# tudocomp/tudocomp

Measured on AMD Instinct MI355X. Metric: input MB/s end-to-end lcpcomp+huffman, higher is better.
Workload: dtype u32; 1 GPU; lcpcomp(coder=huff,threshold=2,flatten=1,comp=arrays) on 2000000000 B english text (SURVEY 8d generator, seed 42): pinned host text -> H2D -> kernels + host Huffman table -> D2H -> stream in pinned host memory, all timed; bytes_per_gpu=2000000000, parallelism=single GPU

## Files before the change

### include/tdc_gpu.h

```cpp
#ifndef TDC_GPU_H
#define TDC_GPU_H

#include <stddef.h>
#include <stdint.h>

#ifdef __cplusplus
extern "C" {
#endif

typedef enum {
    TDC_GPU_OK = 0,
    TDC_GPU_ERR_HIP = -1,
    TDC_GPU_ERR_ARG = -2,
    TDC_GPU_ERR_NO_SENTINEL = -3,
    TDC_GPU_ERR_TOO_LARGE = -4,
    TDC_GPU_ERR_OOM = -5,
    TDC_GPU_ERR_UNSUPPORTED = -6,
    TDC_GPU_ERR_INTERNAL = -7
} tdc_gpu_status;

enum { TDC_GPU_CODER_HUFF = 0, TDC_GPU_CODER_GAMMA = 1, TDC_GPU_CODER_ARITH = 2, TDC_GPU_CODER_ASCII = 3, TDC_GPU_CODER_SLE = 4,
       TDC_GPU_CODER_BIT = 5 , TDC_GPU_CODER_DELTA = 6  };
#define TDC_GPU_CODER_SLE_K(K) (TDC_GPU_CODER_SLE | ((K) << 8))
enum { TDC_GPU_COMP_ARRAYS = 0, TDC_GPU_COMP_PLCPPEAKS = 1, TDC_GPU_COMP_MAXLCP = 2, TDC_GPU_COMP_HEAP = 3 };

typedef struct tdc_gpu_ctx tdc_gpu_ctx;

typedef struct {
    uint64_t n;
    uint64_t out_len;
    uint64_t factors;
    uint64_t maxlcp;
    uint64_t entries;
    uint64_t num_flattened;
    uint64_t max_depth_lb;
    uint64_t flen_min, flen_max, fdist_max;
    uint64_t pushes;
    uint32_t sa_rounds;
    uint32_t sa_init_syms;
    uint32_t levels;
    uint32_t mis_rounds;
    uint32_t flatten_rounds;
    uint32_t sigma;
    uint64_t sa_sorted_elems;
    uint64_t arena_bytes;
    float ms_h2d, ms_sa, ms_phi, ms_plcp, ms_factorize, ms_flatten, ms_encode, ms_d2h, ms_total;
    uint32_t small_levels;
    uint32_t purges;
    uint32_t window_pass;
    uint32_t window_lcut;
    uint32_t sa_key_words;
    uint32_t sa_text_rounds;
    uint32_t sa_mode;
    uint32_t sa_overlapped;
    uint32_t eager_levels;
    uint32_t eager_phases;
    uint32_t sa_star_chains;
    uint32_t probes;
    uint32_t max_push_targets;
    uint64_t d2h_early;
    uint32_t pipe_stages;
    uint32_t pipe_dev;
    uint64_t pipe_len[8];
    float    pipe_ms[8];
    uint32_t ranges_early;
    uint32_t len_rounds;
    uint64_t rules;
    uint64_t replaced;
    uint32_t tie_rounds;
    uint32_t rebuilds;
    float ms_round_first, ms_round_last, ms_round_tie;
    float reserved1;
} tdc_gpu_stats;

int  tdc_gpu_ctx_create(int device, tdc_gpu_ctx** ctx);
void tdc_gpu_ctx_destroy(tdc_gpu_ctx* ctx);
int tdc_gpu_ctx_set_option(tdc_gpu_ctx* ctx, const char* name, long value);
int tdc_gpu_option_count(void);
const char* tdc_gpu_option_name(int i);
int  tdc_gpu_ctx_reserve(tdc_gpu_ctx* ctx, size_t n);
size_t tdc_gpu_arena_bytes(size_t n);
int  tdc_gpu_device_memory(int device, size_t* free_bytes, size_t* total_bytes);
int  tdc_gpu_ctx_set_profiling(tdc_gpu_ctx* ctx, int enabled);
void tdc_gpu_ctx_reset_profile(tdc_gpu_ctx* ctx);
const char* tdc_gpu_ctx_kernel_profile(const tdc_gpu_ctx* ctx, int idx, double* ms, uint64_t* launches, uint64_t* bytes);
const char* tdc_gpu_strerror(int status);
const char* tdc_gpu_last_error(const tdc_gpu_ctx* ctx);
void tdc_gpu_free(void* p);

int tdc_gpu_lcpcomp_compress(tdc_gpu_ctx* ctx, const uint8_t* text, size_t n, uint32_t threshold, int flatten,
                             int coder, uint8_t** out, size_t* out_len, tdc_gpu_stats* stats);
int tdc_gpu_lcpcomp_compress_comp(tdc_gpu_ctx* ctx, const uint8_t* text, size_t n, uint32_t threshold, int flatten, int coder,
                                  int comp, uint8_t** out, size_t* out_len, tdc_gpu_stats* stats);

int tdc_gpu_lcpcomp_compress_into(tdc_gpu_ctx* ctx, const uint8_t* text, size_t n, uint32_t threshold, int flatten, int coder,
                                  int comp, uint8_t* out, size_t out_cap, size_t* out_len, tdc_gpu_stats* stats);
int tdc_gpu_lcpcomp_compress_keep(tdc_gpu_ctx* ctx, const uint8_t* text, size_t n, uint32_t threshold, int flatten, int coder,
                                  int comp, size_t* out_len, tdc_gpu_stats* stats);
int tdc_gpu_stream_fetch(tdc_gpu_ctx* ctx, uint8_t* dst, size_t cap, size_t* len);
int tdc_gpu_stream_fetch_dev(tdc_gpu_ctx* ctx, void* d_dst, size_t cap, size_t* len);
int tdc_gpu_host_register(void* p, size_t bytes);
int tdc_gpu_host_unregister(void* p);
void* tdc_gpu_host_alloc(size_t bytes);
void  tdc_gpu_host_free(void* p);

int tdc_gpu_lcpcomp_compress_raw(tdc_gpu_ctx* ctx, const uint8_t* data, size_t n, uint32_t threshold, int flatten,
                                 int coder, uint8_t** out, size_t* out_len, tdc_gpu_stats* stats);
int tdc_gpu_lcpcomp_compress_dev(tdc_gpu_ctx* ctx, const void* d_text, size_t n, uint32_t threshold, int flatten,
                                 int coder, void* d_out, size_t out_cap, size_t* out_len, tdc_gpu_stats* stats);
size_t tdc_gpu_lcpcomp_bound(size_t n);
size_t tdc_gpu_lcpcomp_bound_coder(size_t n, int coder);

size_t tdc_gpu_blocks_count(size_t n, size_t block_size);
int tdc_gpu_blocks_compress(const int* devices, int ndev, const uint8_t* data, size_t n, size_t block_size, uint32_t threshold,
                            int flatten, int coder, uint8_t** out, size_t* out_len, tdc_gpu_stats* per_block);
int tdc_gpu_blocks_decompress(tdc_gpu_ctx* ctx, const uint8_t* container, size_t len, int coder, uint8_t** out, size_t* out_len);
int tdc_gpu_device_count(void);

int tdc_gpu_lz78_compress(tdc_gpu_ctx* ctx, const uint8_t* in, size_t n, int coder, uint8_t** out, size_t* out_len,
                          tdc_gpu_stats* stats);

int tdc_gpu_lzss_lcp_compress(tdc_gpu_ctx* ctx, const uint8_t* text, size_t n, uint32_t threshold, int coder,
                              uint8_t** out, size_t* out_len, tdc_gpu_stats* stats);
int tdc_gpu_lzss_lcp_compress_into(tdc_gpu_ctx* ctx, const uint8_t* text, size_t n, uint32_t threshold, int coder,
                                   uint8_t* out, size_t out_cap, size_t* out_len, tdc_gpu_stats* stats);
size_t tdc_gpu_lzss_lcp_bound(size_t n, int coder);
int tdc_gpu_lzss_lcp_decompress(tdc_gpu_ctx* ctx, const uint8_t* stream, size_t len, int coder, uint8_t** out, size_t* out_len,
                                uint64_t* factors, uint32_t* rounds);
int tdc_gpu_lzss_lcp_decompress_into(tdc_gpu_ctx* ctx, const uint8_t* stream, size_t len, int coder, uint8_t* out, size_t out_cap,
                                     size_t* out_len, uint64_t* factors, uint32_t* rounds);
int tdc_gpu_lzss_lcp_factorize(tdc_gpu_ctx* ctx, const uint8_t* text, size_t n, uint32_t threshold,
                               uint32_t** pos, uint32_t** src, uint32_t** len, size_t* z);

int tdc_gpu_sort_pairs_u64(tdc_gpu_ctx* ctx, uint64_t* keys, uint32_t* vals, size_t n, int algo);
int tdc_gpu_suffix_array(tdc_gpu_ctx* ctx, const uint8_t* text, size_t n, uint32_t* sa, uint32_t* isa);
int tdc_gpu_textds(tdc_gpu_ctx* ctx, const uint8_t* text, size_t n, uint32_t* sa, uint32_t* isa, uint32_t* phi,
                   uint32_t* plcp, uint32_t* lcp, uint32_t* maxlcp);
int tdc_gpu_lcpcomp_factorize(tdc_gpu_ctx* ctx, const uint8_t* text, size_t n, uint32_t threshold, int flatten,
                              uint32_t** pos, uint32_t** src, uint32_t** len, size_t* z, tdc_gpu_stats* stats);
int tdc_gpu_flatten(tdc_gpu_ctx* ctx, size_t n, const uint32_t* pos, uint32_t* src, const uint32_t* len, size_t z,
                    uint64_t* num_flattened, uint64_t* max_depth_lb);
int tdc_gpu_prim_scan(tdc_gpu_ctx* ctx, int op, void* data, size_t n, int in_place, void* total);
int tdc_gpu_prim_sort_pairs(tdc_gpu_ctx* ctx, int kind, void* keys, uint32_t* vals, size_t n, int begin_bit, int end_bit);
int tdc_gpu_prim_bucketed_scatter(tdc_gpu_ctx* ctx, const uint32_t* idx, const uint32_t* val, size_t m, uint32_t* dst, size_t n_dst,
                                  uint32_t fill, int permutation, int second_tmp, int offset);
int tdc_gpu_prim_msd_partition(tdc_gpu_ctx* ctx, uint32_t* idx, uint32_t* val, size_t m, int bits, int db);
int tdc_gpu_prim_select(tdc_gpu_ctx* ctx, const uint8_t* cls, uint8_t want, size_t m, const uint32_t* srcA, const uint64_t* srcB,
                        uint32_t fillA, uint64_t fillB, uint32_t* outA, uint64_t* outB, uint32_t* count);
int tdc_gpu_prim_select_counts(tdc_gpu_ctx* ctx, const uint8_t* cls, uint8_t want, size_t m, const uint32_t* srcA, const uint32_t* tile_counts,
                               uint32_t fillA, uint32_t* outA, uint32_t* count);
int tdc_gpu_prim_mark_orbit(tdc_gpu_ctx* ctx, const uint32_t* next, size_t n, uint8_t* mark);
int tdc_gpu_prim_tile_entries(tdc_gpu_ctx* ctx, const uint16_t* exit0, size_t ntiles, uint32_t states, uint16_t* entry0);
int tdc_gpu_prim_arena_fill(tdc_gpu_ctx* ctx, int byte, uint64_t* base, uint64_t* size);

int tdc_gpu_lcpcomp_decompress(tdc_gpu_ctx* ctx, const uint8_t* stream, size_t len, uint8_t** out, size_t* out_len,
// ... 133 lines not shown
```

### tudocomp_amd/_native.py

```python
import ctypes
import os

_HERE = os.path.dirname(os.path.abspath(__file__))
LIB_PATH = os.environ.get("TDC_GPU_LIB") or os.path.join(_HERE, "lib", "libtdc_gpu.so")

SYMBOLS = [
    "tdc_gpu_ctx_create", "tdc_gpu_ctx_destroy", "tdc_gpu_ctx_reserve", "tdc_gpu_strerror", "tdc_gpu_last_error",
    "tdc_gpu_ctx_set_profiling", "tdc_gpu_ctx_reset_profile", "tdc_gpu_ctx_kernel_profile",
    "tdc_gpu_free", "tdc_gpu_lcpcomp_compress", "tdc_gpu_lcpcomp_compress_raw", "tdc_gpu_lcpcomp_compress_dev",
    "tdc_gpu_lcpcomp_bound", "tdc_gpu_lcpcomp_bound_coder", "tdc_gpu_lcpcomp_compress_into", "tdc_gpu_host_alloc", "tdc_gpu_host_free",
    "tdc_gpu_lz78_compress", "tdc_gpu_lzss_lcp_compress", "tdc_gpu_lzss_lcp_factorize",
    "tdc_gpu_sort_pairs_u64", "tdc_gpu_suffix_array", "tdc_gpu_textds", "tdc_gpu_lcpcomp_factorize", "tdc_gpu_flatten", "tdc_gpu_encode_huff",
    "tdc_gpu_prim_scan", "tdc_gpu_prim_sort_pairs", "tdc_gpu_prim_bucketed_scatter", "tdc_gpu_prim_msd_partition", "tdc_gpu_prim_select", "tdc_gpu_prim_select_counts",
    "tdc_gpu_prim_mark_orbit", "tdc_gpu_prim_tile_entries", "tdc_gpu_prim_arena_fill",
    "tdc_gpu_lcpcomp_decompress",
    "tdc_gpu_lcpcomp_compress_comp",
    "tdc_gpu_encode_arith",
    "tdc_gpu_encode_ascii",
    "tdc_gpu_encode_sle",
    "tdc_gpu_lcpcomp_decompress_coder", "tdc_gpu_ctx_last_decode_on_device", "tdc_gpu_lcpcomp_decompress_into",
    "tdc_gpu_ctx_set_option", "tdc_gpu_option_count", "tdc_gpu_option_name", "tdc_escape", "tdc_unescape", "tdc_lz78_factors", "tdc_huffman_table", "tdc_huffman_selfcheck", "tdc_gpu_blocks_count", "tdc_gpu_blocks_compress", "tdc_gpu_blocks_decompress", "tdc_gpu_device_count", "tdc_gen_english", "tdc_gen_dna",
    "tdc_gpu_arena_bytes", "tdc_gpu_device_memory",
    "tdc_gpu_lcpcomp_compress_keep", "tdc_gpu_stream_fetch", "tdc_gpu_stream_fetch_dev", "tdc_gpu_host_register", "tdc_gpu_host_unregister",
    "tdc_gpu_lz78_decompress", "tdc_gpu_lz78_decompress_into",
    "tdc_gpu_bwt_compress", "tdc_gpu_bwt_compress_into", "tdc_gpu_bwt_decompress", "tdc_gpu_bwt_decompress_into", "tdc_gpu_bwt_inverse_stage",
    "tdc_gpu_pipeline_bound", "tdc_gpu_pipeline_compress", "tdc_gpu_pipeline_compress_into", "tdc_gpu_pipeline_decompress",
    "tdc_gpu_pipeline_decompress_into", "tdc_gpu_pipeline_decompress_stats", "tdc_rle_decode", "tdc_mtf_decode", "tdc_huff_decode_literals", "tdc_sle_decode",
    "tdc_gpu_lzw_compress", "tdc_gpu_lzw_decompress", "tdc_gpu_lzw_decompress_into", "tdc_lzw_factors", "tdc_lzw_decode",
    "tdc_gpu_lzss_lcp_compress_into", "tdc_gpu_lzss_lcp_bound", "tdc_gpu_lzss_lcp_decompress", "tdc_gpu_lzss_lcp_decompress_into", "tdc_lzss_decode",
    "tdc_gpu_lzss_sw_compress", "tdc_gpu_lzss_sw_compress_into", "tdc_gpu_lzss_sw_bound", "tdc_gpu_lzss_sw_factorize", "tdc_lzss_sw_factors",
    "tdc_lzss_sw_decode", "tdc_gpu_lzss_sw_decompress", "tdc_gpu_lzss_sw_decompress_into",
    "tdc_gpu_lzss_sw_compress_batch", "tdc_gpu_lzss_sw_batch_bound", "tdc_gpu_lzss_sw_decompress_batch",
    "tdc_gpu_lzw_compress_batch", "tdc_gpu_lzw_batch_bound", "tdc_gpu_lz78_compress_batch", "tdc_gpu_lz78_batch_bound", "tdc_gpu_lz_parse_batch",
    "tdc_gpu_lzw_decompress_batch", "tdc_gpu_lz78_decompress_batch",
    "tdc_gpu_repair_compress", "tdc_gpu_repair_compress_into", "tdc_gpu_repair_bound", "tdc_gpu_repair_grammar", "tdc_gpu_repair_decompress",
    "tdc_gpu_repair_decompress_into", "tdc_gpu_repair_decompress_stats", "tdc_repair_grammar", "tdc_repair_decode",
]


class Stats(ctypes.Structure):
    _fields_ = (
        [(k, ctypes.c_uint64) for k in ("n", "out_len", "factors", "maxlcp", "entries", "num_flattened", "max_depth_lb",
                                        "flen_min", "flen_max", "fdist_max", "pushes")] +
        [(k, ctypes.c_uint32) for k in ("sa_rounds", "sa_init_syms", "levels", "mis_rounds", "flatten_rounds", "sigma")] +
        [(k, ctypes.c_uint64) for k in ("sa_sorted_elems", "arena_bytes")] +
        [(k, ctypes.c_float) for k in ("ms_h2d", "ms_sa", "ms_phi", "ms_plcp", "ms_factorize", "ms_flatten", "ms_encode",
                                       "ms_d2h", "ms_total")] +
        [(k, ctypes.c_uint32) for k in ("small_levels", "purges", "window_pass", "window_lcut",
                                        "sa_key_words", "sa_text_rounds", "sa_mode", "sa_overlapped", "eager_levels", "eager_phases", "sa_star_chains",
                                        "probes", "max_push_targets")] +
        [("d2h_early", ctypes.c_uint64)] +
        [("pipe_stages", ctypes.c_uint32), ("pipe_dev", ctypes.c_uint32), ("pipe_len", ctypes.c_uint64 * 8), ("pipe_ms", ctypes.c_float * 8),
         ("ranges_early", ctypes.c_uint32), ("len_rounds", ctypes.c_uint32),
         ("rules", ctypes.c_uint64), ("replaced", ctypes.c_uint64), ("tie_rounds", ctypes.c_uint32), ("rebuilds", ctypes.c_uint32),
         ("ms_round_first", ctypes.c_float), ("ms_round_last", ctypes.c_float), ("ms_round_tie", ctypes.c_float), ("reserved1", ctypes.c_float)])

    def as_dict(self):
        d = {k: getattr(self, k) for k, _ in self._fields_}
        d["pipe_len"] = list(self.pipe_len)[:self.pipe_stages]
        d["pipe_ms"] = list(self.pipe_ms)[:self.pipe_stages]
        return d


class Stage(ctypes.Structure):
    _fields_ = [("kind", ctypes.c_int), ("param", ctypes.c_uint64)]


_lib = None


def load():
    global _lib
    if _lib is not None:
        return _lib
    if not os.path.exists(LIB_PATH):
        raise RuntimeError("tudocomp_amd: %s is missing -- build it with `make -C tudocomp_amd/csrc` "
                           "(there is no CPU fallback)" % LIB_PATH)
    L = ctypes.CDLL(LIB_PATH)
    vp, sz, u32, i32 = ctypes.c_void_p, ctypes.c_size_t, ctypes.c_uint32, ctypes.c_int
    pvp, psz = ctypes.POINTER(vp), ctypes.POINTER(sz)
    L.tdc_gpu_ctx_create.argtypes = [i32, pvp]
    L.tdc_gpu_ctx_destroy.argtypes = [vp]
    L.tdc_gpu_ctx_destroy.restype = None
    L.tdc_gpu_ctx_reserve.argtypes = [vp, sz]
    L.tdc_gpu_ctx_set_profiling.argtypes = [vp, i32]
    L.tdc_gpu_ctx_reset_profile.argtypes = [vp]
    L.tdc_gpu_ctx_reset_profile.restype = None
    L.tdc_gpu_ctx_kernel_profile.argtypes = [vp, i32, ctypes.POINTER(ctypes.c_double), ctypes.POINTER(ctypes.c_uint64),
                                             ctypes.POINTER(ctypes.c_uint64)]
    L.tdc_gpu_ctx_kernel_profile.restype = ctypes.c_char_p
    L.tdc_gpu_strerror.argtypes = [i32]
    L.tdc_gpu_strerror.restype = ctypes.c_char_p
    L.tdc_gpu_last_error.argtypes = [vp]
    L.tdc_gpu_last_error.restype = ctypes.c_char_p
    L.tdc_gpu_free.argtypes = [vp]
    L.tdc_gpu_free.restype = None
    L.tdc_gpu_lcpcomp_compress.argtypes = [vp, vp, sz, u32, i32, i32, pvp, psz, ctypes.POINTER(Stats)]
    L.tdc_gpu_lcpcomp_compress_comp.argtypes = [vp, vp, sz, u32, i32, i32, i32, pvp, psz, ctypes.POINTER(Stats)]
    L.tdc_gpu_lcpcomp_compress_raw.argtypes = [vp, vp, sz, u32, i32, i32, pvp, psz, ctypes.POINTER(Stats)]
    L.tdc_gpu_lcpcomp_compress_dev.argtypes = [vp, vp, sz, u32, i32, i32, vp, sz, psz, ctypes.POINTER(Stats)]
    L.tdc_gpu_lz78_compress.argtypes = [vp, vp, sz, i32, pvp, psz, ctypes.POINTER(Stats)]
    L.tdc_gpu_lzss_lcp_compress.argtypes = [vp, vp, sz, u32, i32, pvp, psz, ctypes.POINTER(Stats)]
    L.tdc_gpu_lzss_lcp_compress_into.argtypes = [vp, vp, sz, u32, i32, vp, sz, psz, ctypes.POINTER(Stats)]
    L.tdc_gpu_lzss_lcp_bound.argtypes = [sz, i32]
    L.tdc_gpu_lzss_lcp_bound.restype = sz
    L.tdc_gpu_lzss_lcp_decompress.argtypes = [vp, vp, sz, i32, pvp, psz, ctypes.POINTER(ctypes.c_uint64), ctypes.POINTER(ctypes.c_uint32)]
    L.tdc_gpu_lzss_lcp_decompress_into.argtypes = [vp, vp, sz, i32, vp, sz, psz, ctypes.POINTER(ctypes.c_uint64), ctypes.POINTER(ctypes.c_uint32)]
    L.tdc_lzss_decode.argtypes = [vp, sz, i32, vp, sz, psz]
    L.tdc_gpu_lzss_lcp_factorize.argtypes = [vp, vp, sz, u32, pvp, pvp, pvp, psz]
    L.tdc_gpu_arena_bytes.argtypes = [sz]
    L.tdc_gpu_arena_bytes.restype = sz
    L.tdc_gpu_device_memory.argtypes = [i32, psz, psz]
    L.tdc_gpu_lcpcomp_bound.argtypes = [sz]
    L.tdc_gpu_lcpcomp_bound.restype = sz
    L.tdc_gpu_lcpcomp_bound_coder.argtypes = [sz, i32]
    L.tdc_gpu_lcpcomp_bound_coder.restype = sz
    L.tdc_gpu_lcpcomp_compress_into.argtypes = [vp, vp, sz, u32, i32, i32, i32, vp, sz, psz, ctypes.POINTER(Stats)]
    L.tdc_gpu_lcpcomp_compress_keep.argtypes = [vp, vp, sz, u32, i32, i32, i32, psz, ctypes.POINTER(Stats)]
    L.tdc_gpu_stream_fetch.argtypes = [vp, vp, sz, psz]
    L.tdc_gpu_stream_fetch_dev.argtypes = [vp, vp, sz, psz]
    L.tdc_gpu_ctx_last_decode_on_device.argtypes = [vp]
    L.tdc_gpu_lcpcomp_decompress_into.argtypes = [vp, vp, sz, i32, vp, sz, psz, ctypes.POINTER(ctypes.c_uint64), ctypes.POINTER(ctypes.c_uint32)]
    L.tdc_gpu_host_register.argtypes = [vp, sz]
    L.tdc_gpu_host_unregister.argtypes = [vp]
    L.tdc_gpu_blocks_count.argtypes = [sz, sz]
    L.tdc_gpu_blocks_count.restype = sz
    L.tdc_gpu_blocks_compress.argtypes = [ctypes.POINTER(i32), i32, vp, sz, sz, u32, i32, i32, pvp, psz, ctypes.POINTER(Stats)]
    L.tdc_gpu_blocks_decompress.argtypes = [vp, vp, sz, i32, pvp, psz]
    L.tdc_gpu_host_alloc.argtypes = [sz]
    L.tdc_gpu_host_alloc.restype = vp
    L.tdc_gpu_host_free.argtypes = [vp]
    L.tdc_gpu_host_free.restype = None
    L.tdc_gpu_sort_pairs_u64.argtypes = [vp, vp, vp, sz, i32]
    L.tdc_gpu_prim_scan.argtypes = [vp, i32, vp, sz, i32, vp]
    L.tdc_gpu_prim_sort_pairs.argtypes = [vp, i32, vp, vp, sz, i32, i32]
    L.tdc_gpu_prim_bucketed_scatter.argtypes = [vp, vp, vp, sz, vp, sz, u32, i32, i32, i32]
    L.tdc_gpu_prim_msd_partition.argtypes = [vp, vp, vp, sz, i32, i32]
    L.tdc_gpu_prim_select.argtypes = [vp, vp, ctypes.c_uint8, sz, vp, vp, u32, ctypes.c_uint64, vp, vp, ctypes.POINTER(u32)]
# ... 83 lines not shown
```

### tudocomp_amd/csrc/api_compress.hip

```cpp
#include "api.hpp"
#include "bitsink.hpp"

#include <vector>

using namespace tdc;

namespace tdc {

void validate_device_text(Ctx& c, const u8* d_text, size_t n) {
    if (!(c.hist_ptr == d_text && c.hist_n == n)) {
        const size_t mark = c.arena.mark();
        u32* d_hist = c.arena.get<u32>(256);
        HIP_TRY(hipMemsetAsync(d_hist, 0, 256 * sizeof(u32), c.stream));
        text_histogram_add(c, d_text, n, d_hist);
        text_histogram_finish(c, d_text, n, d_hist);
        c.arena.release(mark);
    }
    u8 last = 1;
    HIP_TRY(hipMemcpyAsync(&last, d_text + n - 1, 1, hipMemcpyDeviceToHost, c.stream));
    HIP_TRY(hipStreamSynchronize(c.stream));
    const u32 zeros = c.hist_cache[0];
    if (last != 0) throw ArgError{TDC_GPU_ERR_NO_SENTINEL, "text does not end with a 0 sentinel"};
    if (zeros != 1) throw ArgError{TDC_GPU_ERR_ARG, "text contains 0 bytes besides the sentinel (escape the input first)"};
}

static bool early_is_planned(const Ctx& c, size_t n, u32 threshold, int flatten, int strategy, int enc_coder, const u8* d_text) {
    return strategy == TDC_GPU_COMP_ARRAYS && flatten && enc_coder == 0 && d_text && c.enc_early && c.enc_rec && c.huff_ok &&
           n >= (c.enc_early >= 2 ? (size_t)1 : ((size_t)1 << 20)) && threshold >= 2;
}

void run_textds(Ctx& c, const u8* d_text, size_t n, DevArrays& A, tdc_gpu_stats* st, Events* ev, bool want_phi, const CandWant* cw) {
    A.sa = c.arena.get<u32>(n);
    A.isa = c.arena.get<u32>(n);
    A.phi = nullptr;
    A.plcp = c.arena.get<u32>(n);
    u32* d_max = c.arena.get<u32>(1);
    SAStats ss;
    SAExtra ex;
    ex.lcp8 = c.arena.get<u8>(n + 64);
    const int e0 = ev ? ev->tick() : 0;
    build_suffix_array(c, d_text, n, A.sa, A.isa, &ss, &ex);
    const int e1 = ev ? ev->tick() : 0;
    int e2;
    if (!(ex.mode == 1 && !want_phi && c.phi_lazy)) A.phi = c.arena.get<u32>(n);
    if (ex.mode == 1) {
        CandFused* cf = nullptr;
        if (cw && c.fused_cand && !A.phi && fused_scatter_has_image(c, n)) {
            cf = &A.cand;
            cf->threshold = cw->threshold;
            cf->lcut = factorize_arrays_lcut0(c, n, cw->threshold);
            cf->cls = c.arena.get<u8>(n);
            if (cf->lcut) cf->res8 = c.arena.get<u8>(n);
            if (cw->flen8) cf->flen8 = A.fs.flen8 = c.arena.get<u8>(n + 64); else cf->flen = A.fs.flen = c.arena.get<u32>(n);
            if (c.sel_tile_counts) cf->tilecnt = c.arena.get<u32>(cdiv(n, SEL_TILE_CLASSES));
            cf->acc = c.arena.get<u32>((size_t)CF_COPIES * CF_ACC);
            cf->lvlhist = c.arena.get<u32>(128);
            cf->entries = cf->lvlhist + 64;
        }
        build_isa_phi_plcp_fused(c, A.sa, ex.lcp8, n, A.isa, A.phi, A.plcp, d_max, cf);
        e2 = ev ? ev->tick() : 0;
    } else {
        build_phi(c, A.sa, n, A.phi);
        e2 = ev ? ev->tick() : 0;
        build_plcp(c, d_text, n, A.phi, A.plcp, d_max);
    }
    const int e3 = ev ? ev->tick() : 0;
    A.maxlcp = c.read(d_max);
    if (st) {
        st->maxlcp = A.maxlcp;
        sa_stats(st, ss, &ex);
        if (ev) { ev->span(&st->ms_sa, e0, e1); ev->span(&st->ms_phi, e1, e2); ev->span(&st->ms_plcp, e2, e3); }
    }
}

constexpr size_t FLAT_CHUNK_MIN = (size_t)16 << 20;
constexpr size_t FLAT_CHUNK_MAX = 8;

void run_factorize(Ctx& c, size_t n, DevArrays& A, u32 threshold, int flatten, tdc_gpu_stats* st, Events* ev, int strategy,
                   int enc_coder, const u8* d_text) {
    if (!A.fs.flen) A.fs.flen = c.arena.get<u32>(n);
    A.fs.owner = c.arena.get<u32>(n);
    A.fs.fsrc = c.arena.get<u32>(n);
    A.fs.fpos = c.arena.get<u32>(n);
    A.fs.flenl = threshold >= 2 ? A.fs.fpos + (n + 1) / 2 : nullptr;
    A.fs.cls = c.arena.get<u8>(n + 64);
    const bool early_planned = early_is_planned(c, n, threshold, flatten, strategy, enc_coder, d_text);
    if (early_planned && c.flen_bytes && !A.fs.flen8) A.fs.flen8 = c.arena.get<u8>(n + 64);
    A.fs.want_owner_rem = early_planned ? (u32)c.owner_rem : 0u;
    FactorizeStats fz;
    FlattenStats fl;
    const int e0 = ev ? ev->tick() : 0;
    if (strategy == TDC_GPU_COMP_PLCPPEAKS) plcp_peaks_factorize(c, n, A.phi, A.plcp, threshold, A.fs, &fz.factors);
    else if (strategy == TDC_GPU_COMP_MAXLCP) factorize_max_lcp(c, n, A.isa, A.phi, A.plcp, A.maxlcp, threshold, A.fs, &fz);
    else if (strategy == TDC_GPU_COMP_HEAP) factorize_max_heap(c, n, A.sa, A.isa, A.plcp, A.maxlcp, threshold, A.fs, &fz);
    else factorize_arrays(c, n, A.sa, A.isa, A.phi, A.plcp, A.maxlcp, threshold, A.fs, &fz, A.cand.filled ? &A.cand : nullptr);
    const int e1 = ev ? ev->tick() : 0;
    const bool early = flatten && enc_coder == 0 && d_text && c.enc_early && c.huff_ok && n >= (c.enc_early >= 2 ? (size_t)1 : ((size_t)1 << 20)) &&
                       A.fs.have_list && A.fs.have_cls && A.fs.flenl && A.fs.nfact > 0;
    if (!early) expand_flen8(c, n, A.fs);
    if (early) {
        A.early = encode_early_reserve(c, n, c.enc_rec ? A.fs.nfact : 0);
        u32 K = c.flatten_chunks ? (u32)c.flatten_chunks : (u32)std::min<size_t>(A.fs.nfact / FLAT_CHUNK_MIN, FLAT_CHUNK_MAX);
        K = flatten_chunk_count(K, A.fs.nfact);
        const bool packed = K >= 2 && encode_early_chunks(c, n, A.fs, A.early, K, align_up(encode_bound_coder(n, enc_coder) + 16, 8));
        if (!packed && c.flatten_chunks < 2) K = 1;
        c.wait_for(c.copy_stream, c.stream);
        flatten_factors(c, n, A.fs, &fl, [&](int round) {
            StreamSwap sw(c, c.copy_stream);
            if (round == 1 || round == 2) encode_early_run(c, d_text, n, A.fs, enc_coder, A.early, false);
            else if (round == 0) encode_early_run(c, d_text, n, A.fs, enc_coder, A.early, true);
        }, c.enc_rec ? encode_early_rec(A.early) : nullptr, K,
        packed ? std::function<void(u32, size_t)>([&](u32 k, size_t) { encode_early_chunk_done(c, d_text, n, A.fs, A.early, k); }) : std::function<void(u32, size_t)>());
    } else if (flatten) {
        flatten_factors(c, n, A.fs, &fl);
    } else {
        materialize_sources(c, n, A.fs);
    }
    const int e2 = ev ? ev->tick() : 0;
    if (st) {
        st->factors = fz.factors; st->entries = fz.entries; st->pushes = fz.pushes;
        st->levels = fz.levels; st->mis_rounds = fz.rounds; st->small_levels = fz.small_levels; st->purges = fz.purges; st->window_pass = fz.window_pass; st->window_lcut = fz.window_lcut; st->eager_levels = fz.eager_levels; st->eager_phases = fz.eager_phases;
        st->probes = fz.probes; st->max_push_targets = fz.max_push_targets;
        st->num_flattened = fl.num_flattened; st->max_depth_lb = fl.max_depth_lb; st->flatten_rounds = fl.rounds;
        st->ranges_early = A.early ? encode_early_packed(A.early) : 0u;
        if (ev) { ev->span(&st->ms_factorize, e0, e1); ev->span(&st->ms_flatten, e1, e2); }
    }
}

u8* TextUpload::send(const uint8_t* text, size_t n) {
    if (n < ((size_t)1 << 26)) return upload_plain(c, text, n);
    u8* d_text = c.arena.get<u8>(n + 64);
    u32* d_hist = c.arena.get<u32>(256);
    HIP_TRY(hipMemsetAsync(d_hist, 0, 256 * sizeof(u32), c.stream));
    c.wait_for(c.copy_stream, c.stream);
    const bool try_pre = c.wsort_overlap && c.wpre && wsort_applicable(c, n);
    const size_t CH = try_pre ? (size_t)c.upload_chunks : 8;
    std::vector<size_t> coff;
    {
        std::vector<double> w(CH, 1.0);
        if (try_pre) {
            const size_t T = std::min<size_t>((size_t)c.upload_tail_n, CH - 1);
            double f = 1.0;
            for (size_t k = 0; k < T; ++k) { f *= (double)c.upload_tail_pct / 100.0; w[CH - T + k] = f; }
        }
        double tot = 0; for (double x : w) tot += x;
        coff.push_back(0);
        double acc = 0;
        for (size_t k = 0; k + 1 < CH; ++k) {
            acc += w[k];
            size_t o = ((size_t)((double)n * (acc / tot)) + 4095) & ~(size_t)4095;
            if (o <= coff.back()) o = coff.back() + 4096;
            if (o >= n) break;
            coff.push_back(o);
        }
        coff.push_back(n);
    }
    const size_t nch = coff.size() - 1;
    if (nch > Ctx::CHUNK_EVENTS) throw HipError{hipErrorUnknown, "upload: more chunks than chunk events", (int)__LINE__};
    size_t queued = 0;
    auto queue_copies = [&](size_t upto) {
        for (; queued < nch && queued < upto; ++queued) {
            const size_t off = coff[queued] + (queued ? 64 : 0), end = std::min(coff[queued + 1] + 64, n);
            if (end > off) HIP_TRY(hipMemcpyAsync(d_text + off, text + off, end - off, hipMemcpyHostToDevice, c.copy_stream));
            HIP_TRY(hipEventRecord(c.ev_chunk[queued], c.copy_stream));
            (void)hipStreamQuery(c.copy_stream);
        }
    };
    bool pre_on = false;
    for (size_t q = 0; q < nch; ++q) {
        const size_t off = coff[q], len = coff[q + 1] - off;
        queue_copies(q + 4);
        HIP_TRY(hipStreamWaitEvent(c.stream, c.ev_chunk[q], 0));
        text_histogram_add(c, d_text + off, len, d_hist);
        if (q == 0 && try_pre) {
            u32 h0[256];
            c.read_n(d_hist, h0, 256);
            pre_on = wsort_pre_begin(c, *c.wpre, d_text, n, coff.data(), (u32)nch, h0);
            if (!pre_on) c.arena.release_top();
        }
        if (pre_on) wsort_pre_chunk(c, *c.wpre, (u32)q);
    }
    text_histogram_finish(c, d_text, n, d_hist);
    if (pre_on) {
        wsort_pre_finish(c, *c.wpre, c.hist_cache);
        if (!c.wpre->active) c.arena.release_top();
    }
    return d_text;
}

struct HostBuf {
    void* p = nullptr;
    explicit HostBuf(size_t bytes) : p(malloc(bytes ? bytes : 1)) { if (!p) throw std::bad_alloc(); }
    ~HostBuf() { free(p); }
    template <typename T> T* release() { T* r = (T*)p; p = nullptr; return r; }
    HostBuf(const HostBuf&) = delete;
    HostBuf& operator=(const HostBuf&) = delete;
};

void download_factors(Ctx& c, size_t n, const FactorSpace& fs, Events& ev, uint32_t** pos, uint32_t** src, uint32_t** len, size_t* z) {
    u32* d_pos = c.arena.get<u32>(n), *d_src = c.arena.get<u32>(n), *d_len = c.arena.get<u32>(n);
    const size_t cnt = extract_factors(c, n, fs, d_pos, d_src, d_len, n);
    HostBuf hp(cnt * 4), hs(cnt * 4), hl(cnt * 4);
    if (cnt) {
        HIP_TRY(hipMemcpyAsync(hp.p, d_pos, cnt * 4, hipMemcpyDeviceToHost, c.stream));
        HIP_TRY(hipMemcpyAsync(hs.p, d_src, cnt * 4, hipMemcpyDeviceToHost, c.stream));
        HIP_TRY(hipMemcpyAsync(hl.p, d_len, cnt * 4, hipMemcpyDeviceToHost, c.stream));
    }
// ... 623 lines not shown
```

### tudocomp_amd/csrc/api_ctx.hip

```cpp
#include "api.hpp"
#include "huffman_host.hpp"

#include <strings.h>
#include <ctype.h>

using namespace tdc;

namespace tdc {

int lcpcomp_enc_coder(int coder) {
    const int base = coder & 0xFF, k = coder >> 8;
    if (base == TDC_GPU_CODER_SLE) {
        if (k < 0 || k > 7) throw ArgError{TDC_GPU_ERR_ARG, "sle: kmer must be in 1..7"};
        return 3 | ((k ? k : 3) << 8);
    }
    if (k == 0 && base == TDC_GPU_CODER_HUFF) return 0;
    if (k == 0 && base == TDC_GPU_CODER_ARITH) return 1;
    if (k == 0 && base == TDC_GPU_CODER_ASCII) return 2;
    throw ArgError{TDC_GPU_ERR_UNSUPPORTED, "lcpcomp: coder must be huff, arithmetic, ascii or sle"};
}

void reserve_arena(Ctx& c, size_t bytes) {
    if (c.arena.size < bytes) {
        size_t fr = 0, tot = 0;
// ... 25 lines not shown
        default: return "unknown status";
    }
}

const char* tdc_gpu_last_error(const tdc_gpu_ctx* ctx) { return ctx ? ctx->last_error.c_str() : ""; }

void tdc_gpu_free(void* p) { free(p); }

namespace {
struct OptionDef { const char* name; void (*set)(Ctx&, long); };
inline int clampi(long v, long lo, long hi) { return (int)(v < lo ? lo : (v > hi ? hi : v)); }
const OptionDef OPTIONS[] = {
    { "fastread",         [](Ctx& c, long v) { c.fast_read = v ? 1 : 0; } },
    { "sa_local",         [](Ctx& c, long v) { c.sa_local_sort = (int)v; } },
    { "radix_waves",      [](Ctx& c, long v) { c.radix_waves = v == 8 ? 8 : 4; } },
    { "window_lcut",      [](Ctx& c, long v) { c.window_lcut = clampi(v, 0, 63); } },
    { "window_halo",      [](Ctx& c, long v) { c.window_halo = clampi(v, 0, 2048); } },
    { "dec_seg",          [](Ctx& c, long v) { c.dec_seg = v < 4096 ? 4096 : (v > (1l << 30) ? (size_t)1 << 30 : (size_t)v); } },
    { "dec_lean",         [](Ctx& c, long v) { c.dec_lean = v != 0; } },
    { "dec_parse",        [](Ctx& c, long v) { c.dec_parse = clampi(v, 0, 2); } },
    { "dec_done",         [](Ctx& c, long v) { c.dec_done = v != 0; } },
    { "dec_log",          [](Ctx& c, long v) { c.dec_log = v != 0; } },
    { "bwt_log",          [](Ctx& c, long v) { c.bwt_log = v != 0; } },
    { "pipe_log",         [](Ctx& c, long v) { c.pipe_log = v != 0; } },
    { "window_force_fail",[](Ctx& c, long v) { c.window_force_fail = v ? 1 : 0; } },
    { "window_large",     [](Ctx& c, long v) { c.window_large_lists = v ? 1 : 0; } },
    { "window_src",       [](Ctx& c, long v) { c.window_src = v ? 1 : 0; } },
    { "plcp_samples",     [](Ctx& c, long v) { c.plcp_samples = v != 0; } },
    { "small_pipeline",   [](Ctx& c, long v) { c.small_pipeline = v != 0; } },
    { "small_big",        [](Ctx& c, long v) { c.small_big = (int)v; } },
    { "small_prof",       [](Ctx& c, long v) { c.small_prof = v != 0; } },
    { "phi_lazy",         [](Ctx& c, long v) { c.phi_lazy = v != 0; } },
    { "fs_pair",          [](Ctx& c, long v) { c.fs_pair = v != 0; } },
    { "enc_early",        [](Ctx& c, long v) { c.enc_early = (int)v; } },
    { "owner_rem",        [](Ctx& c, long v) { c.owner_rem = (int)std::min<long>(std::max<long>(v, 0), 8); } },
    { "enc_rec",          [](Ctx& c, long v) { c.enc_rec = v != 0; } },
    { "level_purge",      [](Ctx& c, long v) { c.level_purge = v != 0; } },
    { "level_log",        [](Ctx& c, long v) { c.level_log = v != 0; } },
    { "eager",            [](Ctx& c, long v) { c.eager_levels = v != 0; } },
    { "eager_dump",       [](Ctx& c, long v) { c.eager_dump = v != 0; } },
    { "flen_bytes",       [](Ctx& c, long v) { c.flen_bytes = v != 0; } },
    { "flatten_steps",    [](Ctx& c, long v) { c.flatten_steps = v <= 0 ? (1 << 30) : clampi(v, 1, 1 << 30); } },
    { "flatten_growth",   [](Ctx& c, long v) { c.flatten_growth = clampi(v, 2, 1 << 20); } },
    { "sa_refine",        [](Ctx& c, long v) { c.sa_refine = v != 0; } },
    { "sa_pairs",         [](Ctx& c, long v) { c.sa_pairs = v != 0; } },
    { "sa_stars",         [](Ctx& c, long v) { c.sa_stars = v != 0; } },
    { "sa_fused_init",    [](Ctx& c, long v) { c.sa_fused_init = v != 0; } },
    { "sa_init_syms",     [](Ctx& c, long v) { c.sa_init_syms = clampi(v, 0, 64); } },
    { "radix_lds",        [](Ctx& c, long v) { c.radix_lds = (v >= 0 && v <= 2) ? (int)v : 2; } },
    { "xcd_remap",        [](Ctx& c, long v) { c.xcd_remap = (v >= 0 && v <= 2) ? (int)v : 0; } },
    { "bucket_scatter",   [](Ctx& c, long v) { c.bucket_scatter = v ? 1 : 0; } },
    { "ssort",            [](Ctx& c, long v) { c.ssort = v ? 1 : 0; } },
    { "ssort_levels",     [](Ctx& c, long v) { c.ssort_levels = (v >= 1 && v <= 3) ? (int)v : 0; } },
    { "msd_partition",    [](Ctx& c, long v) { c.msd_partition = v ? 1 : 0; } },
    { "wsort",            [](Ctx& c, long v) { c.wsort = v ? 1 : 0; } },
    { "wsort_min",        [](Ctx& c, long v) { c.wsort_min = v < 4096 ? 4096 : (size_t)v; } },
    { "wsort_syms",       [](Ctx& c, long v) { c.wsort_syms = (v >= 4 && v <= 64) ? (int)v : 0; } },
    { "wsort_kw",         [](Ctx& c, long v) { c.wsort_kw = (v == 1 || v == 2) ? (int)v : 0; } },
    { "wsort_rounds",     [](Ctx& c, long v) { c.wsort_rounds = clampi(v, 0, 100); } },
    { "wsort_smallrun",   [](Ctx& c, long v) { c.wsort_small = v ? 1 : 0; } },
    { "wsort_overlap",    [](Ctx& c, long v) { c.wsort_overlap = v ? 1 : 0; } },
    { "wsort_predig",     [](Ctx& c, long v) { c.wsort_predig = v ? 1 : 0; } },
    { "wsort_prehist",    [](Ctx& c, long v) { c.wsort_prehist = v ? 1 : 0; } },
    { "sa_seg_bigcap",    [](Ctx& c, long v) { c.sa_seg_bigcap = clampi(v, 0, 65536); } },
    { "sa_seg_rounds",    [](Ctx& c, long v) { c.sa_seg_rounds = clampi(v, 0, 2); } },
    { "wsort_run_streams",[](Ctx& c, long v) { c.wsort_run_streams = v != 0; } },
    { "wsort_predig_skip",[](Ctx& c, long v) { c.wsort_predig_skip = clampi(v, 0, 24); } },
    { "wsort_fuse",       [](Ctx& c, long v) { c.wsort_fuse = v ? 1 : 0; } },
    { "wsort_order",      [](Ctx& c, long v) { c.wsort_order = v ? 1 : 0; } },
    { "wsort_two",        [](Ctx& c, long v) { c.wsort_two = (v >= 0 && v <= 2) ? (int)v : 0; } },
    { "wsort_leaf",       [](Ctx& c, long v) { c.wsort_leaf = v == 1024 ? 1024 : 2048; } },
    { "wsort_pack",       [](Ctx& c, long v) { c.wsort_pack = (v == 1024 || v == 4096) ? (int)v : 2048; } },
    { "wsort_cmax",       [](Ctx& c, long v) { c.wsort_cmax = clampi(v, 8, 64); } },
    { "wsort_log",        [](Ctx& c, long v) { c.wsort_log = v != 0; } },
    { "upload_chunks",    [](Ctx& c, long v) { c.upload_chunks = clampi(v, 4, 24); } },
    { "upload_tail_n",    [](Ctx& c, long v) { c.upload_tail_n = clampi(v, 0, 12); } },
    { "upload_tail_pct",  [](Ctx& c, long v) { c.upload_tail_pct = clampi(v, 30, 100); } },
    { "arena_log",        [](Ctx& c, long v) { c.arena_log = v != 0; } },
};
constexpr size_t NOPTIONS = sizeof(OPTIONS) / sizeof(OPTIONS[0]);
const OptionDef FOLD_OPTIONS[] = {
    { "fused_cand",       [](Ctx& c, long v) { c.fused_cand = v != 0; } },
    { "sel_tile_counts",  [](Ctx& c, long v) { c.sel_tile_counts = v != 0; } },
    { "flatten_chunks",   [](Ctx& c, long v) { c.flatten_chunks = clampi(v, 0, (long)FLATTEN_MAX_CHUNKS); } },
    { "repair_recount",   [](Ctx& c, long v) { c.repair_recount = v != 0; } },
    { "repair_table_bits",[](Ctx& c, long v) { c.repair_table_bits = v == 0 ? 0 : clampi(v, 8, 30); } },
    { "repair_log",       [](Ctx& c, long v) { c.repair_log = v != 0; } },
    { "repair_dec_rounds",[](Ctx& c, long v) { c.repair_dec_rounds = clampi(v, 1, 1 << 24); } },
    { "lz_batch_hash_bits",[](Ctx& c, long v) { c.lz_batch_hash_bits = clampi(v, 0, 24); } },
};
constexpr size_t NFOLD = sizeof(FOLD_OPTIONS) / sizeof(FOLD_OPTIONS[0]);
const OptionDef* find_option(const char* name) {
    if (!name) return nullptr;
    if (!strncasecmp(name, "TDC_GPU_", 8)) name += 8;
    for (size_t i = 0; i < NOPTIONS; ++i) if (!strcasecmp(name, OPTIONS[i].name)) return &OPTIONS[i];
    for (size_t i = 0; i < NFOLD; ++i) if (!strcasecmp(name, FOLD_OPTIONS[i].name)) return &FOLD_OPTIONS[i];
    return nullptr;
}
void apply_env_options(tdc_gpu_ctx* ctx) {
    const char* on = getenv("TDC_GPU_DEBUG_KNOBS");
    if (!on || atoi(on) == 0) return;
    for (size_t i = 0; i < NOPTIONS + NFOLD; ++i) {
        const OptionDef& o = i < NOPTIONS ? OPTIONS[i] : FOLD_OPTIONS[i - NOPTIONS];
        char var[64] = "TDC_GPU_";
        size_t k = 8;
        for (const char* q = o.name; *q && k + 1 < sizeof(var); ++q) var[k++] = (char)toupper((unsigned char)*q);
        var[k] = 0;
        if (const char* m = getenv(var)) o.set(ctx->c, atol(m));
    }
}
}

int tdc_gpu_ctx_set_option(tdc_gpu_ctx* ctx, const char* name, long value) {
    if (!ctx) return TDC_GPU_ERR_ARG;
    const OptionDef* o = find_option(name);
    if (!o) return TDC_GPU_ERR_ARG;
    o->set(ctx->c, value);
    return TDC_GPU_OK;
}
int tdc_gpu_option_count(void) { return (int)NOPTIONS; }
const char* tdc_gpu_option_name(int i) { return (i >= 0 && (size_t)i < NOPTIONS) ? OPTIONS[i].name : nullptr; }

int tdc_gpu_ctx_create(int device, tdc_gpu_ctx** out) {
    if (!out) return TDC_GPU_ERR_ARG;
    *out = nullptr;
    int count = 0;
    if (hipGetDeviceCount(&count) != hipSuccess || count <= 0) { (void)hipGetLastError(); return TDC_GPU_ERR_HIP; }
    if (device < 0 || device >= count) return TDC_GPU_ERR_ARG;
    tdc_gpu_ctx* ctx = new (std::nothrow) tdc_gpu_ctx();
    if (!ctx) return TDC_GPU_ERR_OOM;
    ctx->c.huff_ok = huffman_selfcheck();
    ctx->c.device = device;
    ctx->c.wpre = &ctx->pre;
    DeviceGuard dg(device);
    try {
        HIP_TRY(dg.enter());
        HIP_TRY(hipStreamCreateWithFlags(&ctx->c.stream, hipStreamNonBlocking));
        for (auto& e : ctx->c.ev) HIP_TRY(hipEventCreate(&e));
        HIP_TRY(hipStreamCreateWithFlags(&ctx->c.copy_stream, hipStreamNonBlocking));
        {
            int lo = 0, hi = 0;
            if (hipDeviceGetStreamPriorityRange(&lo, &hi) != hipSuccess) { lo = 0; (void)hipGetLastError(); }
            if (hipStreamCreateWithPriority(&ctx->c.aux_stream, hipStreamNonBlocking, lo) != hipSuccess) { ctx->c.aux_stream = nullptr; (void)hipGetLastError(); }
        }
        HIP_TRY(hipEventCreateWithFlags(&ctx->c.ev_join, hipEventDisableTiming));
        HIP_TRY(hipEventCreateWithFlags(&ctx->c.ev_dig2, hipEventDisableTiming));
        for (auto& e : ctx->c.ev_chunk) HIP_TRY(hipEventCreateWithFlags(&e, hipEventDisableTiming));
        ctx->c.pinned_size = 4096;
        HIP_TRY(hipHostMalloc(&ctx->c.pinned, ctx->c.pinned_size, hipHostMallocDefault));
        HIP_TRY(hipHostMalloc((void**)&ctx->c.pinned_hdr, Ctx::PINNED_HDR, hipHostMallocDefault));
        if (ctx->c.fast_read) {
            void* zc = nullptr;
            if (hipHostMalloc(&zc, (size_t)Ctx::ZC_WORDS * Ctx::ZC_BLOCKS * 4, hipHostMallocMapped | hipHostMallocCoherent) == hipSuccess) {
                void* dv = nullptr;
                if (hipHostGetDevicePointer(&dv, zc, 0) == hipSuccess) { ctx->c.zc_host = (u32*)zc; ctx->c.zc_dev = (u32*)dv; memset(zc, 0, (size_t)Ctx::ZC_WORDS * Ctx::ZC_BLOCKS * 4); }
                else { (void)hipHostFree(zc); (void)hipGetLastError(); }
            } else (void)hipGetLastError();
        }
        HIP_TRY(hipMalloc((void**)&ctx->c.d_err, 256));
        HIP_TRY(hipMemset(ctx->c.d_err, 0, 256));
        apply_env_options(ctx);
    } catch (const HipError&) {
        (void)hipGetLastError();
        tdc_gpu_ctx_destroy(ctx);
        return TDC_GPU_ERR_HIP;
    }
    *out = ctx;
// ... 141 lines not shown
```

### tudocomp_amd/csrc/common.hpp

```cpp
#pragma once

#include <hip/hip_runtime.h>
#include <stdint.h>
#include <stddef.h>
#include <stdio.h>
#include <string.h>

namespace tdc {

typedef uint8_t  u8;
typedef uint32_t u32;
typedef uint16_t u16;
typedef uint64_t u64;

constexpr u32 NONE32 = 0xFFFFFFFFu;
constexpr int WAVE = 64;

enum {
    TDC_OK = 0,
    TDC_ERR_HIP = -1,
    TDC_ERR_ARG = -2,
    TDC_ERR_NO_SENTINEL = -3,
    TDC_ERR_TOO_LARGE = -4,
    TDC_ERR_OOM = -5,
// ... 34 lines not shown
        if (top > high) high = top;
        return base + off;
    }
    template <typename T> T* get(size_t count) { return (T*)alloc(count * sizeof(T)); }
    void* alloc_top(size_t bytes) {
        if (bytes + top_hi + 256 > size) throw HipError{hipErrorOutOfMemory, "arena (top)", (int)__LINE__};
        const size_t off = (size - top_hi - bytes) & ~(size_t)255;
        if (off < top) throw HipError{hipErrorOutOfMemory, "arena (top)", (int)__LINE__};
        top_hi = size - off;
        return base + off;
    }
    template <typename T> T* get_top(size_t count) { return (T*)alloc_top(count * sizeof(T)); }
    void release_top() { top_hi = 0; }
    size_t mark() const { return top; }
    void release(size_t m) { top = m; }
};

enum KernelClass {
    K_RS_SCATTER_U64 = 0, K_RS_SCATTER_U32, K_RS_COUNT, K_SCAN,
    K_SA_RANK_SCATTER, K_SA_BUILD_KEYS, K_PHI, K_PLCP, K_CAND,
    K_LEVEL_INIT, K_MIS_ROUND, K_RESOLVE, K_PUSH, K_APPLY, K_POOL, K_SMALL_LEVEL, K_WINDOW_LEVELS,
    K_FLATTEN_ROUND, K_ENC_GAPS, K_ENC_HIST, K_ENC_TILE_BITS, K_ENC_PACK, K_EXTRACT, K_SS_LEAF, K_SA_LOCAL_SORT, K_WINDOW_SCATTER,
    K_WS_LEAF_SORT, K_WS_LEAF_COUNT, K_WS_RUN, K_FS_IMAGE,
    K_CLASS_COUNT
};

struct KernelProfile {
    double ms = 0;
    u64 launches = 0;
    u64 bytes = 0;
};

#ifdef __HIPCC__
static __global__ void publish_words_kernel(const uint32_t* __restrict__ src, uint32_t nwords, uint32_t* host_dst, uint32_t* host_flag,
                                            uint32_t seq) {
    for (uint32_t i = threadIdx.x; i < nwords; i += blockDim.x)
        __hip_atomic_store(&host_dst[i], src[i], __ATOMIC_RELAXED, __HIP_MEMORY_SCOPE_SYSTEM);
    __syncthreads();
    if (threadIdx.x == 0) {
        __threadfence_system();
        __hip_atomic_store(host_flag, seq, __ATOMIC_RELEASE, __HIP_MEMORY_SCOPE_SYSTEM);
    }
}
#endif

struct Ctx {
    int device = 0;
    hipStream_t stream = nullptr;
    Arena arena;
    hipEvent_t ev[16] = {};
    void* pinned = nullptr;
    size_t pinned_size = 0;
    void* pinned_tab = nullptr;
    size_t pinned_tab_size = 0;
    u8* pinned_hdr = nullptr;
    static constexpr size_t PINNED_HDR = 65536;
    void* pinned_table(size_t bytes) {
        if (pinned_tab_size < bytes) {
            if (pinned_tab) { (void)hipHostFree(pinned_tab); pinned_tab = nullptr; pinned_tab_size = 0; }
            HIP_TRY(hipHostMalloc(&pinned_tab, bytes, hipHostMallocDefault));
            pinned_tab_size = bytes;
        }
        return pinned_tab;
    }
    static constexpr u32 ZC_SEG_OFF = 1040, ZC_WORDS = 1040 + 16384;
    static constexpr u32 ZC_BLOCKS = 3;
    u32* zc_host = nullptr;
    u32* zc_dev = nullptr;
    u32 zc_seq = 0;
    int fast_read = 1;
    u32* d_err = nullptr;
    int sa_local_sort = 1;
    int radix_waves = 4;
    int plcp_samples = 1;
    bool huff_ok = true;
    int flen_bytes = 1;
    int eager_levels = 1;
    int level_purge = 1;
    int enc_rec = 1;
    int owner_rem = 8;
    int enc_early = 1;
    int fused_cand = 1;
    int sel_tile_counts = 1;
    int fs_pair = 1;
    int small_big = 1;
    int small_pipeline = 1;
    int sa_pairs = 1;
    int sa_stars = 1;
    int sa_refine = 1;
    int sa_fused_init = 1;
    int radix_lds = 1;
    int xcd_remap = 1;
    int window_src = 1;
    int window_lcut = 56;
    int window_halo = 320;
    size_t dec_seg = 0;
    bool phi_lazy = true;
    int dec_lean = 1;
    int dec_parse = 1;
    int window_force_fail = 0;
    int window_large_lists = 0;
    int ssort = 1;
    int ssort_levels = 0;
    int wsort = 1;
    size_t wsort_min = (size_t)1 << 20;
    int wsort_syms = 0;
    int wsort_kw = 0;
    int wsort_rounds = 24;
    int wsort_cmax = 24;
    int wsort_overlap = 1;
    int wsort_prehist = 1;
    bool wsort_count_nonheads = true;
    int sa_seg_bigcap = 65536;
    int sa_seg_rounds = 2;
    int wsort_run_streams = 1;
    int wsort_predig_skip = 4;
    int wsort_predig = 1;
    int wsort_two = 0;
    int wsort_leaf = 2048;
    int wsort_pack = 1024;
    int wsort_order = 1;
    int wsort_fuse = 1;
    int wsort_small = 0;
    int msd_partition = 1;
    int bucket_scatter = 1;
    int upload_tail_n = 3, upload_tail_pct = 60;
    int upload_chunks = 16;
    int flatten_steps = 1;
    int flatten_growth = 8;
    int flatten_chunks = 0;
    int sa_init_syms = 0;
    int dec_done = 1;
    int repair_recount = 0;
    int repair_table_bits = 0;
    int repair_log = 0;
    int repair_dec_rounds = 1024;
    int lz_batch_hash_bits = 0;
    int dec_log = 0, bwt_log = 0, pipe_log = 0, level_log = 0, wsort_log = 0, eager_dump = 0, small_prof = 0, arena_log = 0;

    u32 hist_cache[256] = {};
    const u8* hist_ptr = nullptr;
    size_t hist_n = 0;
    hipStream_t copy_stream = nullptr;
    hipStream_t aux_stream = nullptr;
    hipEvent_t ev_join = nullptr;
    static constexpr size_t CHUNK_EVENTS = 32;
    hipEvent_t ev_chunk[CHUNK_EVENTS] = {};
    hipEvent_t ev_dig2 = nullptr;
    struct WPre* wpre = nullptr;
    u8* d2h_host = nullptr;
    size_t d2h_cap = 0;
    size_t d2h_done = 0;

    bool profiling = false;
    KernelProfile kprof[K_CLASS_COUNT];
    struct Pending { hipEvent_t a, b; int cls; u64 bytes; };
    Pending* pend = nullptr;
    int npend = 0, pend_cap = 0;
    hipEvent_t* ev_pool = nullptr;
    int ev_pool_size = 0, ev_pool_used = 0;

    int prof_begin(int cls, u64 bytes) {
        if (!profiling || npend >= pend_cap || ev_pool_used + 2 > ev_pool_size) return -1;
        Pending& p = pend[npend];
        p.a = ev_pool[ev_pool_used++]; p.b = ev_pool[ev_pool_used++]; p.cls = cls; p.bytes = bytes;
        HIP_TRY(hipEventRecord(p.a, stream));
// ... 291 lines not shown
```

### tudocomp_amd/csrc/encode.hip

```cpp
#include "stages.hpp"
#include "bytestages.hpp"
#include "bitsink.hpp"
#include "prim.hpp"
#include "huffman_host.hpp"
#include "arith.hpp"
#include "decode.hpp"

#include <string.h>
#include <algorithm>
#include <vector>

namespace tdc {

struct CodeTable {
    u64 code[256];
    u8 len[256];
};

struct EncParams {
    u32 W, lbits, dbits, flen_min;
    u32 raw_literals;
    u32 ascii;
    u32 uni;
};
// ... 498 lines not shown
        build_huffman_table(h_hist, &ht);
        write_huffman_header(hw, ht);
    } else {
        ArithModel am;
        if (!arith_build_model(h_hist, &am, hw))
            throw HipError{hipErrorInvalidValue, "arithmetic coder: all literal bytes >= 1 are absent (the reference divides by zero)", -1};
        ArithPlan plan;
        arith_prepare(c, text, n, plain_owner(fs), am, &plan);
        E.A.litidx = plan.litidx; E.A.amark = plan.amark; E.A.fval = plan.fval; E.A.lc_index = plan.lc_index; E.A.pp_lb = plan.pp_lb;
    }
    EncParams& P = E.P;
    P.W = bits_for(n);
    P.lbits = bits_for((u64)h_sc.flen_max - (u64)h_sc.flen_min);
    P.dbits = bits_for(h_sc.fdist_max);
    P.flen_min = h_sc.flen_min;
    P.raw_literals = (ht.sigma <= 1) ? 1u : 0u;
    P.ascii = (coder == 2) ? 1u : 0u;
    P.uni = coder == 5 ? (u32)ENC_GAMMA : coder == 6 ? (u32)ENC_DELTA : 0u;
    if (P.uni) {
        const u64 fields[4] = { (u64)n, h_sc.flen_min, h_sc.flen_max, h_sc.fdist_max };
        auto gamma = [&](u64 v) { const unsigned b = bits_for(v); hw.write_int(0, b); hw.write_bit(true); hw.write_int(v, b); };
        for (u64 v : fields) {
            if (P.uni == (u32)ENC_GAMMA) gamma(v);
            else { gamma(bits_for(v)); hw.write_int(v, bits_for(v)); }
        }
    } else if (coder == 2) {
        const u64 fields[4] = { (u64)n, h_sc.flen_min, h_sc.flen_max, h_sc.fdist_max };
        for (u64 v : fields) {
            char tmp[24]; int k = 0;
            do { tmp[k++] = (char)('0' + v % 10); v /= 10; } while (v);
            while (k) hw.write_int((u8)tmp[--k], 8);
            hw.write_int(':', 8);
        }
    } else {
        hw.write_int(n, 32);
        hw.write_int(h_sc.flen_min, P.W);
        hw.write_int(h_sc.flen_max, P.W);
        hw.write_int(h_sc.fdist_max, P.W);
    }
    E.base_bits = hw.nbits;
    memcpy(E.tab.code, ht.code_of, sizeof(E.tab.code));
    memcpy(E.tab.len, ht.len_of, sizeof(E.tab.len));

    const unsigned tiles = E.tiles;
    u64* tile_bits = E.tile_bits;
    {
        Ctx::ProfScope prof(c, K_ENC_TILE_BITS, (u64)n * 9);
        if (P.uni == (u32)ENC_GAMMA) tile_bits_kernel<ENC_GAMMA><<<tiles, 256, 0, s>>>(text, plain_owner(fs), fs.flen, fs.fsrc, n, E.tab, P, E.A, tile_bits);
        else if (P.uni == (u32)ENC_DELTA) tile_bits_kernel<ENC_DELTA><<<tiles, 256, 0, s>>>(text, plain_owner(fs), fs.flen, fs.fsrc, n, E.tab, P, E.A, tile_bits);
        else if (P.ascii) tile_bits_kernel<ENC_ASCII><<<tiles, 256, 0, s>>>(text, plain_owner(fs), fs.flen, fs.fsrc, n, E.tab, P, E.A, tile_bits);
        else if (fs.have_cls) tile_bits_cls_kernel<<<tiles, 256, 0, s>>>(text, fs.cls, n, E.tab, P, E.A, tile_bits, E.tile_rank);
        else         tile_bits_kernel<ENC_TAB><<<tiles, 256, 0, s>>>(text, plain_owner(fs), fs.flen, fs.fsrc, n, E.tab, P, E.A, tile_bits);
        LAUNCH_CHECK();
    }
    exclusive_sum_u64(c, tile_bits, tile_bits, tiles, E.d_tp);
    if (E.tile_rank) exclusive_sum_u32(c, E.tile_rank, E.tile_rank, tiles, nullptr);
    E.may_overlap = may_overlap(c, E);
    pick_u64_kernel<<<1, 64, 0, s>>>(tile_bits, E.end, E.nb, E.d_tp + 1);
    LAUNCH_CHECK();
    E.seq_b = c.publish_async(E.d_tp, (1 + PACK_CH) * sizeof(u64), 2);
    E.step = 2;
}

static void encode_step_c(Ctx& c, EncodeEarly& E) {
    u64 h_tp[1 + PACK_CH] = { 0 };
    if (E.seq_b) c.publish_wait(E.seq_b, h_tp, sizeof(h_tp), 2); else c.read_n(E.d_tp, h_tp, 1 + PACK_CH);
    const bool may_overlap = E.may_overlap;
    E.total_bits = E.base_bits + h_tp[0];
    E.out_len = bit_stream_len(E.total_bits);
    E.overlap = may_overlap && E.out_len <= c.d2h_cap;
    for (u32 q = 0; q < PACK_CH; ++q) E.h_end[q] = h_tp[1 + q];
    E.step = 3;
    E.done = true;
}

static void encode_first_half(Ctx& c, const u8* text, size_t n, FactorSpace& fs, int coder, EncodeEarly& E, bool finish = true) {
    do {
        if (E.step == 0) encode_step_a(c, text, n, fs, E);
        else if (E.step == 1) encode_step_b(c, text, n, fs, coder, E);
        else if (E.step == 2) encode_step_c(c, E);
    } while (finish && E.step < 3);
}

EncodeEarly* encode_early_reserve(Ctx& c, size_t n, size_t z_rec) {
    EncodeEarly* E = new EncodeEarly();
    try { encode_reserve(c, n, *E, z_rec); } catch (...) { delete E; throw; }
    return E;
}
void* encode_early_rec(EncodeEarly* E) { return E->rec; }
void encode_early_run(Ctx& c, const u8* text, size_t n, FactorSpace fs, int coder, EncodeEarly* E, bool finish) { encode_first_half(c, text, n, fs, coder, *E, finish); }
void encode_early_free(EncodeEarly* E) { delete E; }

static void pack_begin(Ctx& c, hipStream_t ps, EncodeEarly& E, u8* d_out) {
    if (E.begun) return;
    const HostBitWriter& hw = E.hw;
    HIP_TRY(hipMemsetAsync(d_out, 0, bit_stream_padded(E.out_len), ps));
    if (c.pinned_hdr && hw.bytes.size() <= Ctx::PINNED_HDR) {
        memcpy(c.pinned_hdr, hw.bytes.data(), hw.bytes.size());
        HIP_TRY(hipMemcpyAsync(d_out, c.pinned_hdr, hw.bytes.size(), hipMemcpyHostToDevice, ps));
    } else HIP_TRY(hipMemcpyAsync(d_out, hw.bytes.data(), hw.bytes.size(), hipMemcpyHostToDevice, ps));
    E.begun = true;
}
static void pack_upto(Ctx& c, hipStream_t ps, hipStream_t cs, const u8* text, size_t n, const FactorSpace& fs, EncodeEarly& E, u8* d_out, u32 upto) {
    if (upto <= E.q_done) return;
    const EncParams& P = E.P;
    const ArithDev& A = E.A;
    const CodeTable& tab = E.tab;
    const u64 base_bits = E.base_bits;
    const u64* tile_bits = E.tile_bits;
    const u32 t0 = E.q_done ? E.end.end[E.q_done - 1] : 0u, t1 = upto == E.nb ? E.tiles : E.end.end[upto - 1];
    if (t1 > t0) {
        if (P.uni == (u32)ENC_GAMMA) pack_kernel<ENC_GAMMA><<<t1 - t0, 256, 0, ps>>>(text, plain_owner(fs), fs.flen, fs.fsrc, n, tab, P, A, tile_bits, base_bits, (u64*)d_out, t0);
        else if (P.uni == (u32)ENC_DELTA) pack_kernel<ENC_DELTA><<<t1 - t0, 256, 0, ps>>>(text, plain_owner(fs), fs.flen, fs.fsrc, n, tab, P, A, tile_bits, base_bits, (u64*)d_out, t0);
        else if (P.ascii) pack_kernel<ENC_ASCII><<<t1 - t0, 256, 0, ps>>>(text, plain_owner(fs), fs.flen, fs.fsrc, n, tab, P, A, tile_bits, base_bits, (u64*)d_out, t0);
        else if (fs.have_cls && E.rec) pack_cls_kernel<true><<<t1 - t0, 256, 0, ps>>>(text, fs.cls, fs.flen, fs.fsrc, n, tab, P, A, tile_bits, base_bits, (u64*)d_out, t0, E.rec, E.tile_rank, (u32)E.z_rec);
        else if (fs.have_cls) pack_cls_kernel<false><<<t1 - t0, 256, 0, ps>>>(text, fs.cls, fs.flen, fs.fsrc, n, tab, P, A, tile_bits, base_bits, (u64*)d_out, t0, nullptr, nullptr, 0u);
        else         pack_kernel<ENC_TAB><<<t1 - t0, 256, 0, ps>>>(text, plain_owner(fs), fs.flen, fs.fsrc, n, tab, P, A, tile_bits, base_bits, (u64*)d_out, t0);
        LAUNCH_CHECK();
    }
    E.q_done = upto;
    if (E.overlap && upto < E.nb) {
        const size_t safe = (size_t)((base_bits + E.h_end[upto - 1]) / 64) * 8;
        bool room = true;
        if (E.by_rank && E.ncopy >= PACK_AHEAD) room = hipEventQuery(c.ev_chunk[PACK_CH + E.ncopy - PACK_AHEAD]) == hipSuccess;
        if (safe > E.copied && room) {
            c.wait_for(cs, ps);
            HIP_TRY(hipMemcpyAsync(c.d2h_host + E.copied, d_out + E.copied, safe - E.copied, hipMemcpyDeviceToHost, cs));
            if (E.by_rank) {
                HIP_TRY(hipEventRecord(c.ev_chunk[PACK_CH + E.ncopy++], cs));
                (void)hipStreamQuery(cs);
            }
            E.copied = safe;
        }
    }
}

bool encode_early_chunks(Ctx& c, size_t n, const FactorSpace& fs, EncodeEarly* e, u32 K, size_t out_cap) {
    EncodeEarly& E = *e;
    const size_t z = fs.nfact;
    if (K < 2 || K > FLATTEN_MAX_CHUNKS || K > z || !fs.have_list || !E.rec || E.z_rec != z || E.step != 0 || !c.aux_stream || !c.pinned_hdr || !may_overlap(c, E)) return false;
    E.d_out = c.arena.get<u8>(out_cap);
    E.out_cap = out_cap;
    u32 h[FLATTEN_MAX_CHUNKS] = { 0 };
    const size_t mark = c.arena.mark();
    u32* d_b = c.arena.get<u32>(FLATTEN_MAX_CHUNKS);
    range_tiles_kernel<<<1, 64, 0, c.stream>>>(fs.fpos, (u32)z, K, d_b);
    LAUNCH_CHECK();
    c.read_n(d_b, h, K - 1);
    c.arena.release(mark);
    for (u32 k = 0; k + 1 < K; ++k) E.end.end[k] = std::min<u32>(h[k], E.tiles);
    for (u32 k = K - 1; k < PACK_CH; ++k) E.end.end[k] = E.tiles;
    E.nb = K;
    E.by_rank = true;
    return true;
}
u8* encode_early_out(EncodeEarly* e, size_t* out_cap) { if (e->d_out && out_cap) *out_cap = e->out_cap; return e->d_out; }
u32 encode_early_packed(const EncodeEarly* e) { return e->by_rank ? e->q_done : 0u; }

void encode_early_chunk_done(Ctx& c, const u8* text, size_t n, const FactorSpace& fs, EncodeEarly* e, u32 k) {
    EncodeEarly& E = *e;
    if (!E.by_rank || k >= E.nb) return;
    HIP_TRY(hipEventRecord(c.ev_chunk[k], c.stream));
    E.q_ready = k + 1;
    if (E.step == 2 && E.seq_b && c.publish_test(E.seq_b, 2)) encode_step_c(c, E);
    if (!E.done || bit_stream_padded(E.out_len) > E.out_cap) return;
    if (E.q_ready == E.nb) return;
    const hipStream_t ps = c.copy_stream, cs = c.aux_stream;
    pack_begin(c, ps, E, E.d_out);
    HIP_TRY(hipStreamWaitEvent(ps, c.ev_chunk[k], 0));
// ... 616 lines not shown
```

### tudocomp_amd/csrc/factorize.hip

```cpp
#include "stages.hpp"
#include "prim.hpp"
#include "factorize_tiles.hpp"
#include "factorize_eager.hpp"

#include <algorithm>
#include <map>
#include <unordered_map>
#include <chrono>
#include <stdlib.h>
#include <vector>

namespace tdc {

enum : u8 { CL_DEAD = 0, CL_LIVE = 1, CL_STALE = 2 };

struct PushSeg { u32 target, start; };
struct GatherSeg { u32 src_off, dst_off; };
constexpr u32 SEG_INLINE = 508;

struct SmallCtl { u32 pool_top, prio_base; };

struct LevelScalars {
    u32 nlive, nstale;
    u32 undecided;
// ... 869 lines not shown
    const u32 i = blockIdx.x * blockDim.x + threadIdx.x;
    if (i >= npush) return;
    const u32 tgt = (u32)(keys[i] >> 32);
    const u32 p = vals[i];
    prio[p] = prio_base + i;
    pool[i] = p;
    if (res8) res8[p] = res8_pushed(tgt);
    if (i == 0 || (u32)(keys[i - 1] >> 32) != tgt) {
        const u32 j = atomicAdd(&sc->nseg, 1u);
        if (j < SEG_INLINE) sc->segs[j] = PushSeg{tgt, i};
        if (j < seg_cap) segs[j] = PushSeg{tgt, i};
    }
}

template <int G>
__global__ __launch_bounds__(256) void apply_kernel(const u32* __restrict__ live, u32 nl, u32 L, size_t n, u64* bm,
                                                     const u32* phi, u32* __restrict__ cur, u32* __restrict__ flen,
                                                     u32* fsrc, LevelScalars* __restrict__ sc, u8* __restrict__ res8, u8* __restrict__ flen8) {
    const u32 i = (blockIdx.x * blockDim.x + threadIdx.x) / G;
    const u32 sub = (G == 1) ? 0u : (threadIdx.x & (G - 1));
    bool sel = false;
    u32 p = 0;
    if (i < nl) { p = live[i]; sel = (bm_state(bm, p) == 2u); }
    if (sel) {
        if (sub == 0) { put_flen(flen, flen8, p, L); if (phi != fsrc) fsrc[p] = phi[p]; }
        for (u32 j = sub; j < L && (size_t)p + j < n; j += G) cur[p + j] = 0;
        const u32 aff = (L < p) ? L : p;
        for (u32 j = sub; j < aff; j += G) {
            u32* q = &cur[p - 1 - j];
            if (*q > j + 1) { if (atomicMin(q, j + 1) > j + 1 && res8) res8[p - 1 - j] = res8_mark(j + 1); }
        }
    }
    if (G > 1) __builtin_amdgcn_wave_barrier();
    if (sel && sub == 0) atomicAnd((unsigned long long*)&bm[p >> 5], ~(3ull << (2 * (p & 31))));
    __shared__ u32 cnt;
    if (threadIdx.x == 0) cnt = 0;
    __syncthreads();
    const u64 b = __ballot(sel && sub == 0);
    if (lane_id() == 0 && b) atomicAdd(&cnt, (u32)__popcll(b));
    __syncthreads();
    if (threadIdx.x == 0 && cnt) atomicAdd(&sc->selected, cnt);
}

u32 factorize_arrays_lcut0(const Ctx& c, size_t n, u32 threshold) {
    if (c.window_lcut <= 0 || n < window_levels_min_text()) return 0;
    const u32 lcut = std::min<u32>((u32)c.window_lcut, window_levels_max_lcut());
    return lcut < threshold ? 0u : lcut;
}

void factorize_arrays(Ctx& c, size_t n, const u32* sa, u32* isa, const u32* phi, u32* plcp, u32 maxlcp, u32 threshold,
                      FactorSpace& fs, FactorizeStats* st, const CandFused* cf) {
    const u32* phi_eff = phi ? phi : fs.fsrc;
    FactorizeStats local;
    if (!st) st = &local;
    *st = FactorizeStats();
    st->maxlcp = maxlcp;
    if (n == 0) return;
    hipStream_t s = c.stream;
    const size_t mark = c.arena.mark();
    const unsigned gn = cdiv(n, 256);
    u32* cur = plcp;
    u32* prio = isa;

    const bool pre = cf && cf->filled;
    if (pre && (phi || cf->threshold != threshold || cf->lcut != factorize_arrays_lcut0(c, n, threshold) || (fs.flen8 ? cf->flen8 != fs.flen8 : cf->flen != fs.flen)))
        throw HipError{hipErrorUnknown, "factorize: the pre-classified candidates belong to another call", (int)__LINE__};
    u8* cls = pre ? cf->cls : c.arena.get<u8>(n);
    u32 lcut = factorize_arrays_lcut0(c, n, threshold);
    if (lcut > maxlcp) lcut = maxlcp;
    if (lcut < threshold) lcut = 0;
    u8* res8 = lcut ? (pre ? cf->res8 : c.arena.get<u8>(n)) : nullptr;
    u32* ckeys[2] = { c.arena.get<u32>(n), c.arena.get<u32>(n) };
    u32* cvals[2] = { c.arena.get<u32>(n), c.arena.get<u32>(n) };
    u32* d_cnt = c.arena.get<u32>(4);
    u32* d_lvlhist = pre ? cf->lvlhist : c.arena.get<u32>(64);
    if (!pre) {
        HIP_TRY(hipMemsetAsync(d_cnt, 0, 4 * sizeof(u32), s));
        HIP_TRY(hipMemsetAsync(d_lvlhist, 0, 64 * sizeof(u32), s));
        Ctx::ProfScope prof(c, K_CAND, (u64)n * (lcut ? 10 : 9) - (fs.flen8 ? (u64)n * 3 : 0));
        cand_class_kernel<<<(gn < 8192u ? gn : 8192u), 256, 0, s>>>(plcp, n, threshold, lcut, cls, fs.flen, res8, d_cnt + 1, lcut ? d_lvlhist : nullptr,
                                                                    phi ? nullptr : sa, isa, fs.fsrc, fs.flen8);
        LAUNCH_CHECK();
    }
    if ((u64)maxlcp + 1 <= threshold || threshold == 0) { c.arena.release(mark); build_owner(c, n, fs); if (!phi) { fs.src_prio = prio; fs.src_sa = sa; fs.src_n = n; } return; }
    const size_t nlev = (size_t)maxlcp + 2;
    u64* rkey = c.arena.get<u64>(n + 2);
    u32* d_segstart = (u32*)rkey;
    u32* d_segend = d_segstart + nlev;
    std::vector<u32> h_segstart(nlev), h_segend(nlev);
    int x = 0;
    size_t cand_count = 0;
    bool first_lists = true;
    auto build_lists = [&](u32 max_level) {
        const bool from_image = pre && first_lists;
        first_lists = false;
        select_by_class(c, cls, 1, n, nullptr, cvals[0], nullptr, nullptr, d_cnt, from_image && c.sel_tile_counts ? cf->tilecnt : nullptr);
        cand_count = c.read(d_cnt);
        if (from_image && !phi && cand_count) {
            Ctx::ProfScope prof(c, K_CAND, (u64)cand_count * 16);
            cand_source_kernel<<<cdiv(cand_count, 256), 256, 0, s>>>(cvals[0], cand_count, sa, isa, n, fs.fsrc);
            LAUNCH_CHECK();
        }
        if (cand_count) {
            Ctx::ProfScope prof(c, K_CAND, (u64)cand_count * 12);
            gather_kernel<<<cdiv(cand_count, 256), 256, 0, s>>>(cvals[0], cand_count, plcp, ckeys[0]);
            LAUNCH_CHECK();
        }
        x = radix_sort_pairs_u32(c, ckeys, cvals, cand_count, 0, (int)bits_for(max_level));
        HIP_TRY(hipMemsetAsync(d_segstart, 0, nlev * sizeof(u32), s));
        HIP_TRY(hipMemsetAsync(d_segend, 0, nlev * sizeof(u32), s));
        if (cand_count) {
            seg_bounds_kernel<<<cdiv(cand_count, 256), 256, 0, s>>>(ckeys[x], cand_count, d_segstart, d_segend);
            LAUNCH_CHECK();
        }
        c.read_n(d_segstart, h_segstart.data(), nlev);
        c.read_n(d_segend, h_segend.data(), nlev);
    };
    build_lists(maxlcp);
    st->entries = c.read(pre ? cf->entries : d_cnt + 1);
    const u32* cand = cvals[x];

    u32* ent = c.arena.get<u32>(n);
    u32* live = c.arena.get<u32>(n);
    u32* stale = c.arena.get<u32>(n);
    const size_t bm_words = n / 32 + 2;
    u64* bm = c.arena.get<u64>(bm_words);
    HIP_TRY(hipMemsetAsync(bm, 0, bm_words * sizeof(u64), s));
    u8* rc = c.arena.get<u8>(n);
    u32* pool = c.arena.get<u32>(n);
    u32* pushed = c.arena.get<u32>(n);
    u32* rval = c.arena.get<u32>(n);
    u64* skeys[2] = { c.arena.get<u64>(n), c.arena.get<u64>(n) };
    u32* svals[2] = { c.arena.get<u32>(n), c.arena.get<u32>(n) };
    LevelScalars* d_sc = (LevelScalars*)c.arena.alloc(sizeof(LevelScalars));
    LevelScalars* d_sc2[2] = { d_sc, (LevelScalars*)c.arena.alloc(sizeof(LevelScalars)) };
    SmallCtl* d_ctl = (SmallCtl*)c.arena.alloc(sizeof(SmallCtl));
    const u32 seg_cap = 1u << 16;
    PushSeg* d_segs = (PushSeg*)c.arena.alloc(sizeof(PushSeg) * seg_cap);
    PushSeg* d_segs2[2] = { d_segs, (PushSeg*)c.arena.alloc(sizeof(PushSeg) * seg_cap) };
    u32 force_general_level = NONE32;
    std::vector<PushSeg> h_segs(seg_cap);
    LevelScalars h_sc;

    const u32 gtab_cap = 1u << 16;
    GatherSeg* d_gtab = (GatherSeg*)c.arena.alloc(sizeof(GatherSeg) * gtab_cap);
    GatherSeg* h_gtab = (GatherSeg*)c.pinned_table(sizeof(GatherSeg) * gtab_cap);
    GatherSeg* d_hgtab = nullptr;
    if (hipHostGetDevicePointer((void**)&d_hgtab, h_gtab, 0) != hipSuccess) { d_hgtab = nullptr; (void)hipGetLastError(); }
    struct PoolSeg { u32 off, cnt; };
    struct LevelLists {
        std::vector<std::vector<PoolSeg>> flat;
        std::unordered_map<u32, std::vector<PoolSeg>> m;
        void init(size_t levels) { if (levels <= ((size_t)1 << 20)) flat.resize(levels); }
        const std::vector<PoolSeg>& get(u32 lv) const {
            static const std::vector<PoolSeg> none;
            if (!flat.empty()) return lv < flat.size() ? flat[lv] : none;
            if (m.empty()) return none;
            auto it = m.find(lv);
            return it == m.end() ? none : it->second;
        }
        std::vector<PoolSeg>& operator[](u32 lv) { return !flat.empty() ? flat[lv] : m[lv]; }
        void drop(u32 lv) {
            if (!flat.empty()) { if (lv < flat.size()) std::vector<PoolSeg>().swap(flat[lv]); }
            else m.erase(lv);
        }
    } pushed_into;
    pushed_into.init((size_t)maxlcp + 2);
// ... 60 lines not shown
        force_general_level = NONE32;
    };
    const u32 eager_floor = std::max<u32>(threshold, lcut ? lcut + 1 : 0);
    const bool eager_possible = c.eager_levels && res8 && nlev <= ((size_t)1 << 22) && maxlcp > eager_floor + 256 && n <= ((size_t)1 << 31);
    u32 eager_phases = 0, small_lazy_streak = 0;
    u32* d_eseg = !eager_possible ? nullptr : (levels_outside ? level_tables.p + nlev : c.arena.get<u32>(2 * nlev));
    u32* d_ehead = eager_possible ? c.arena.get<u32>(nlev) : nullptr;
    EagerCtl* d_ectl = eager_possible ? (EagerCtl*)c.arena.alloc(sizeof(EagerCtl)) : nullptr;
    auto run_eager = [&](u32 Lfrom) -> u32 {
        {
            Ctx::ProfScope prof(c, K_CAND, (u64)n * 6);
            eager_heads_class(c, cur, n, eager_floor - 1, Lfrom, cls);
        }
        select_by_class(c, cls, 1, n, nullptr, ent, nullptr, nullptr, d_cnt);
        const size_t tcount = c.read(d_cnt);
        u32* tk[2] = { live, stale };
        u32* tv[2] = { ent, rval };
        int y = 0;
        HIP_TRY(hipMemsetAsync(d_eseg, 0, 2 * nlev * sizeof(u32), s));
        if (tcount) {
            gather_kernel<<<cdiv(tcount, 256), 256, 0, s>>>(ent, tcount, cur, live);
            LAUNCH_CHECK();
            y = radix_sort_pairs_u32(c, tk, tv, tcount, 0, (int)bits_for(Lfrom));
            seg_bounds_kernel<<<cdiv(tcount, 256), 256, 0, s>>>(tk[y], tcount, d_eseg, d_eseg + nlev);
            LAUNCH_CHECK();
        }
        HIP_TRY(hipMemsetAsync(d_ehead, 0, nlev * sizeof(u32), s));
        HIP_TRY(hipMemsetAsync(d_ectl, 0, sizeof(EagerCtl), s));
        EagerParams P;
        P.tcand = tv[y]; P.tstart = d_eseg; P.tend = d_eseg + nlev;
        P.head = d_ehead;
        P.blk = pool; P.blk_cap = (u32)std::min<size_t>(n / 16, (size_t)1 << 28);
        P.cur = cur; P.prio = prio; P.phi = phi_eff; P.flen = fs.flen; P.flen8 = fs.flen8; P.fsrc = fs.fsrc; P.res8 = res8;
        P.n = n; P.threshold = threshold; P.L_from = Lfrom; P.L_stop = eager_floor; P.raw_cap = eager_levels_raw_cap();
        P.ctl = d_ectl;
        P.dbg = nullptr;
        const size_t dbg_mark = c.arena.mark();
        if (level_log) { P.dbg = c.arena.get<u32>(4 * nlev); HIP_TRY(hipMemsetAsync(P.dbg, 0, 4 * nlev * sizeof(u32), s)); }
        {
            Ctx::ProfScope prof(c, K_SMALL_LEVEL, (u64)tcount * 13 + (u64)(Lfrom - eager_floor + 1) * 16);
            eager_levels_launch(c, P);
        }
        EagerCtl h;
        HIP_TRY(hipMemcpyAsync(&h, d_ectl, sizeof(EagerCtl), hipMemcpyDeviceToHost, s));
        HIP_TRY(hipStreamSynchronize(s));
        if (P.dbg) {
            std::vector<u32> dv(4 * nlev);
            HIP_TRY(hipMemcpy(dv.data(), P.dbg, 4 * nlev * sizeof(u32), hipMemcpyDeviceToHost));
            unsigned long long tot = 0;
            for (size_t lv = 0; lv < nlev; ++lv) tot += dv[4 * lv + 2];
            unsigned long long acc = 0; u32 shown = 0;
            const bool dump_all = c.eager_dump != 0;
            for (size_t lv = nlev; lv-- > 0;) {
                if (!dv[4 * lv + 2]) continue;
                if (dump_all) { fprintf(stderr, "eager level %zu: entries %u factors %u cycles %u\n", lv, dv[4 * lv], dv[4 * lv + 1], dv[4 * lv + 2]); continue; }
                acc += dv[4 * lv + 2];
                if (dv[4 * lv + 2] > 400000u || (shown++ % 256) == 0) fprintf(stderr, "eager level %zu: %u entries of %u candidates, %u factors, %u cycles (running %.1f %% of %llu)\n", lv, dv[4 * lv], dv[4 * lv + 3], dv[4 * lv + 1], dv[4 * lv + 2], 100.0 * (double)acc / (double)(tot ? tot : 1), tot);
            }
            c.arena.release(dbg_mark);
        }
        st->factors += h.factors;
        st->levels += h.levels_done;
        st->small_levels += h.levels_done;
        st->eager_levels += h.levels_done;
        ++eager_phases;
        st->eager_phases = eager_phases;
        if (level_log) fprintf(stderr, "eager phase %u: levels %u .. %u, %u processed, %llu factors, %zu heads at the start, %u blocks, status %u\n",
                               eager_phases, Lfrom, h.level + 1, h.levels_done, h.factors, tcount, h.nblk, h.status);
        return h.level;
    };
    auto t_prev = std::chrono::steady_clock::now();
    for (u32 L = maxlcp; L >= threshold; --L) {
        if (lcut && L == lcut) {
            u64 nf = 0;
            bool start_large = false;
            {
                u32 hh[64];
                c.read_n(d_lvlhist, hh, 64);
                u64 mx = 0;
                for (u32 v = threshold; v <= lcut && v < 64u; ++v) mx = std::max<u64>(mx, hh[v]);
                start_large = (double)mx * 16.0 * (double)window_levels_window() / (double)n > 4.0 * (double)window_levels_small_list();
            }
            const bool wsrc = !phi && c.window_src;
            const int why = factorize_window_levels(c, n, cur, prio, res8, phi, lcut, threshold, fs, &nf, start_large, wsrc ? sa : nullptr);
            const bool ok = why == 0;
            if (ok && wsrc) window_src_done = true;
            st->window_pass = ok ? 1 : 2;
            st->window_lcut = lcut;
            if (ok) { st->factors += nf; break; }
            rebuild_from_cur(threshold - 1, L);
            eager_phases = 99;
            lcut = (why == 1 && L > 24 && threshold <= 24) ? 24 : 0;
        }
        if (eager_possible && eager_phases < 4 && L > eager_floor + 256 && small_lazy_streak >= 4 && L != force_general_level) {
            const bool small_ahead = true;
            if (small_ahead) {
                const u32 next = run_eager(L);
                small_lazy_streak = 0;
                if (next >= eager_floor && next >= threshold) rebuild_from_cur(eager_floor - 1, next);
                else { for (u32 v = eager_floor; v <= L; ++v) pushed_into.drop(v); }
                L = next + 1;
                continue;
            }
        }
        if ((dead_streak >= 4 && levels_since_purge >= 16) || purge_pays) {
            purge_pays = false;
            size_t cnt = 0;
            for (u32 v = L;; --v) { if (h_segend[v] > h_segstart[v]) { cnt = h_segend[v]; break; } if (v == threshold) break; }
            if (cnt > 65536) {
                purge_class_kernel<<<cdiv(cnt, 256), 256, 0, s>>>(cvals[x], cnt, threshold, cur, cls);
                LAUNCH_CHECK();
                select_by_class(c, cls, 1, cnt, cvals[x], cvals[x ^ 1], nullptr, nullptr, d_cnt);
                select_by_class(c, cls, 1, cnt, ckeys[x], ckeys[x ^ 1], nullptr, nullptr, d_cnt);
                x ^= 1;
                cand = cvals[x];
                cand_count = c.read(d_cnt);
                HIP_TRY(hipMemsetAsync(d_segstart, 0, ((size_t)L + 1) * sizeof(u32), s));
                HIP_TRY(hipMemsetAsync(d_segend, 0, ((size_t)L + 1) * sizeof(u32), s));
                if (cand_count) {
                    seg_bounds_kernel<<<cdiv(cand_count, 256), 256, 0, s>>>(ckeys[x], cand_count, d_segstart, d_segend);
                    LAUNCH_CHECK();
                }
                c.read_n(d_segstart, h_segstart.data(), (size_t)L + 1);
                c.read_n(d_segend, h_segend.data(), (size_t)L + 1);
                st->purges++;
                HIP_TRY(hipMemsetAsync(d_lcount, 0xFF, nlev * sizeof(u32), s));
                purge_next = 0xFFFFFFFFu;
            }
            levels_since_purge = 0;
            dead_streak = 0;
        }
        ++levels_since_purge;
        const bool trigger_stale = nolive_run >= stale_trigger;
        if ((probe_dead && (pushed_into.get(L).empty() || dead_levels_run >= 8)) || trigger_stale) {
            const u32 floor_level = std::max<u32>(threshold, lcut ? lcut + 1 : 0);
            const bool deep = dead_levels_run >= 8 || trigger_stale;
            std::vector<ProbeSeg> ptab;
            u32 Lb = L;
            size_t lo = (size_t)-1, hi = 0, cnt = 0;
            for (u32 v = L;; --v) {
                const std::vector<PoolSeg>& pv = pushed_into.get(v);
                if (!pv.empty()) {
                    if (v != L && (!deep || ptab.size() + pv.size() > ((size_t)4 << 20))) break;
                    for (const PoolSeg& sg : pv) ptab.push_back(ProbeSeg{sg.off, sg.cnt, v});
                }
                if (h_segend[v] > h_segstart[v]) {
                    cnt += h_segend[v] - h_segstart[v];
                    if (cnt > ((size_t)4 << 20) && v != L) break;
                    lo = std::min(lo, (size_t)h_segstart[v]); hi = std::max(hi, (size_t)h_segend[v]);
                }
                Lb = v;
                if (v == floor_level) break;
            }
            if (Lb < L) {
                u32 alive = 0, livecur = 0;
                const size_t pmark = c.arena.mark();
                ProbeSeg* d_ptab = nullptr;
                if (hi > lo || !ptab.empty()) {
                    HIP_TRY(hipMemsetAsync(d_cnt + 2, 0, 2 * sizeof(u32), s));
                    u32* d_maxcur = trigger_stale ? d_cnt + 3 : nullptr;
                    if (hi > lo) {
                        unsigned g = cdiv(hi - lo, 256 * 4); if (g > 4096) g = 4096; if (g == 0) g = 1;
                        alive_max_level_kernel<<<g, 256, 0, s>>>(ckeys[x], cvals[x], lo, hi, cur, threshold, d_cnt + 2, d_maxcur);
                        LAUNCH_CHECK();
                    }
                    if (!ptab.empty()) {
                        d_ptab = (ProbeSeg*)c.arena.alloc(ptab.size() * sizeof(ProbeSeg));
                        HIP_TRY(hipMemcpyAsync(d_ptab, ptab.data(), ptab.size() * sizeof(ProbeSeg), hipMemcpyHostToDevice, s));
                        unsigned g = cdiv(ptab.size(), 256); if (g > 4096) g = 4096;
// ... 316 lines not shown
                undecided = now;
            }
        }
        {
            Ctx::ProfScope prof(c, K_RESOLVE, (u64)(ns + nl) * (25 + 8ull * ((2 * L - 2) / 32 + 2)));
            u32* app = mid ? &d_sc->npush : nullptr;
            u64* rk = mid ? skeys[0] : rkey;
            u32* rv = mid ? svals[0] : rval;
            if (ns) {
                if (wide) resolve_kernel<64><<<gs, 256, 0, s>>>(stale, ns, false, L, threshold, n, prio, bm, cur, rk, rv, rc, app);
                else      resolve_kernel<1><<<gs, 256, 0, s>>>(stale, ns, false, L, threshold, n, prio, bm, cur, rk, rv, rc, app);
                LAUNCH_CHECK();
            }
            if (nl) {
                const size_t o = mid ? 0 : ns;
                if (wide) resolve_kernel<64><<<gl, 256, 0, s>>>(live, nl, true, L, threshold, n, prio, bm, cur, rk + o, rv + o, rc + o, app);
                else      resolve_kernel<1><<<gl, 256, 0, s>>>(live, nl, true, L, threshold, n, prio, bm, cur, rk + o, rv + o, rc + o, app);
                LAUNCH_CHECK();
            }
        }
        if (!mid) select_by_class(c, rc, 1, (size_t)ns + nl, rval, svals[0], rkey, skeys[0], &d_sc->npush);
        if (nl) {
            Ctx::ProfScope prof(c, K_APPLY, (u64)nl * 5 + (u64)nl * (12 + 12ull * L));
            if (wide) apply_kernel<64><<<gl, 256, 0, s>>>(live, nl, L, n, bm, phi_eff, cur, fs.flen, fs.fsrc, d_sc, res8, fs.flen8);
            else      apply_kernel<1><<<gl, 256, 0, s>>>(live, nl, L, n, bm, phi_eff, cur, fs.flen, fs.fsrc, d_sc, res8, fs.flen8);
            LAUNCH_CHECK();
        }
        c.read_n((const u32*)d_sc, (u32*)&h_sc, 8);
        st->factors += h_sc.selected;
        const u32 npush = h_sc.npush;
        const u32 rounds_before = st->rounds;
        (void)rounds_before;
        if (npush) {
            if (pool_top + npush > n || (u64)prio_base + npush > 0xFFFFFFFFull)
                throw HipError{hipErrorUnknown, "factorize: push pool overflow", (int)__LINE__};
            const int y = sort_pairs_u64_distinct(c, skeys, svals, npush, 0, 32 + (int)bits_for(L));
            {
                Ctx::ProfScope prof(c, K_PUSH, (u64)npush * 24);
                push_finalize_kernel<<<cdiv(npush, 256), 256, 0, s>>>(skeys[y], svals[y], npush, prio_base, prio,
                                                                      pool + pool_top, res8, d_segs, seg_cap, d_sc);
                LAUNCH_CHECK();
            }
            c.read_n((const u32*)d_sc, (u32*)&h_sc, sizeof(LevelScalars) / sizeof(u32));
            const u32 nseg = h_sc.nseg;
            if (nseg > seg_cap) throw HipError{hipErrorUnknown, "factorize: too many push targets in one level", (int)__LINE__};
            st->max_push_targets = std::max(st->max_push_targets, nseg);
            if (nseg <= SEG_INLINE) std::copy(h_sc.segs, h_sc.segs + nseg, h_segs.begin());
            else c.read_n(d_segs, h_segs.data(), nseg);
            std::sort(h_segs.begin(), h_segs.begin() + nseg, [](const PushSeg& a, const PushSeg& b) { return a.start < b.start; });
            for (u32 j = 0; j < nseg; ++j) {
                const u32 end = (j + 1 < nseg) ? h_segs[j + 1].start : npush;
                const u32 tgt = h_segs[j].target;
                if (tgt >= L || tgt < threshold) throw HipError{hipErrorUnknown, "factorize: bad push target", (int)__LINE__};
                pushed_into[tgt].push_back(PoolSeg{(u32)pool_top + h_segs[j].start, end - h_segs[j].start});
            }
            pool_top += npush;
            prio_base += npush;
            st->pushes += npush;
        }
        if (level_log) {
            const auto t_now = std::chrono::steady_clock::now();
            fprintf(stderr, "level %u m0 %u m1 %u live %u stale %u selected %u npush %u ms %.3f\n", L, m0, m1, nl, ns, h_sc.selected, npush,
                    std::chrono::duration<double, std::milli>(t_now - t_prev).count());
            t_prev = t_now;
        }
        if (L == 0) break;
    }
    if (d_sprof) {
        unsigned long long hh[32];
        HIP_TRY(hipMemcpyAsync(hh, d_sprof, sizeof(hh), hipMemcpyDeviceToHost, s));
        HIP_TRY(hipStreamSynchronize(s));
        if (host_prof[4] > 0)
            fprintf(stderr, "small levels, host side, us per level: prepare %.1f launch %.1f wait %.1f bookkeeping %.1f\n", host_prof[0] / host_prof[4],
                    host_prof[1] / host_prof[4], host_prof[2] / host_prof[4], host_prof[3] / host_prof[4]);
        for (int part = 0; part < 2; ++part) {
            const unsigned long long* h = hh + 16 * part;
            const double lv = h[8] ? (double)h[8] : 1.0;
            fprintf(stderr, "small levels with %s survivors: %llu; per level: raw %.0f alive %.1f selected %.2f pushes %.1f; us (100 MHz clock): load %.1f sort %.1f "
                            "classify %.1f select %.1f push %.1f apply %.1f publish %.1f\n", part ? "> 1024" : "<= 1024", h[8], h[9] / lv, h[10] / lv, h[11] / lv,
                    h[12] / lv, h[0] / 100.0 / lv, h[1] / 100.0 / lv, h[2] / 100.0 / lv, h[3] / 100.0 / lv, h[4] / 100.0 / lv, h[5] / 100.0 / lv, h[6] / 100.0 / lv);
        }
    }
    c.arena.release(mark);
    build_owner(c, n, fs); if (!phi && !window_src_done) { fs.src_prio = prio; fs.src_sa = sa; fs.src_n = n; }
}

__global__ void mlcp_init_prio_kernel(u32* __restrict__ prio, size_t n) {
    const size_t p = (size_t)blockIdx.x * blockDim.x + threadIdx.x;
    if (p < n) prio[p] = 0x80000000u + (u32)(n - 1 - prio[p]);
}
__global__ void mlcp_classify_kernel(const u32* __restrict__ orig, u32 m0, const u32* __restrict__ pushed, u32 m, u32 L,
                                     const u32* __restrict__ cur, u32* __restrict__ live, u64* __restrict__ bm, LevelScalars* __restrict__ sc) {
    const u32 k = blockIdx.x * blockDim.x + threadIdx.x;
    u32 p = 0;
    bool is_live = false;
    if (k < m) { p = (k < m0) ? orig[k] : pushed[k - m0]; is_live = cur[p] == L; }
    const u32 il = wave_append(is_live, &sc->nlive);
    if (is_live) { live[il] = p; atomicOr((unsigned long long*)&bm[p >> 5], 1ull << (2 * (p & 31))); }
}
__global__ void mlcp_collect_kernel(const u32* __restrict__ live, u32 nl, const u32* __restrict__ prio, u64* bm,
                                    u64* __restrict__ skey, u32* __restrict__ sval, LevelScalars* __restrict__ sc) {
    const u32 i = blockIdx.x * blockDim.x + threadIdx.x;
    u32 p = 0;
    bool sel = false;
    if (i < nl) { p = live[i]; sel = bm_state(bm, p) == 2u; }
    const u32 o = wave_append(sel, &sc->selected);
    if (sel) {
        skey[o] = prio[p]; sval[o] = p;
        atomicAnd((unsigned long long*)&bm[p >> 5], ~(3ull << (2 * (p & 31))));
    }
}
template <int G>
__global__ __launch_bounds__(256) void mlcp_apply_kernel(const u32* __restrict__ sel, u32 nsel, u32 L, size_t n, const u32* __restrict__ phi,
                                                          u32* __restrict__ cur, u32* __restrict__ flen, u32* __restrict__ fsrc,
                                                          u32* __restrict__ stamp) {
    const u32 i = (blockIdx.x * blockDim.x + threadIdx.x) / G;
    const u32 sub = (G == 1) ? 0u : (threadIdx.x & (G - 1));
    if (i >= nsel) return;
    const u32 p = sel[i];
    if (sub == 0) { flen[p] = L; fsrc[p] = phi[p]; }
    for (u32 j = sub; j < L && (size_t)p + j < n; j += G) cur[p + j] = 0;
    const u32 aff = (L < p) ? L : p;
    for (u32 j = sub; j < aff; j += G) {
        u32* q = &cur[p - 1 - j];
        if (*q > j + 1) { if (atomicMin(q, j + 1) > j + 1) stamp[p - 1 - j] = L; }
    }
}
template <int G>
__global__ __launch_bounds__(256) void mlcp_push_kernel(const u32* __restrict__ sel, u32 nsel, u32 L, u32 threshold, u32 tbase,
                                                         const u32* __restrict__ cur, const u32* __restrict__ stamp, u32* __restrict__ prio,
                                                         u64* __restrict__ bkey, LevelScalars* __restrict__ sc) {
    const u32 i = (blockIdx.x * blockDim.x + threadIdx.x) / G;
    const u32 sub = (G == 1) ? 0u : (threadIdx.x & (G - 1));
    if (i >= nsel) return;
    const u32 p = sel[i];
    const u32 aff = (L < p) ? L : p;
    for (u32 j = sub; j < aff; j += G) {
        const u32 sp = p - 1 - j, d = j + 1;
        if (d >= threshold && stamp[sp] == L && cur[sp] == d) {
            prio[sp] = 0x7FFFFFFFu - (tbase + i);
            bkey[atomicAdd(&sc->npush, 1u)] = ((u64)d << 32) | sp;
        }
    }
}
__global__ void mlcp_pool_kernel(const u64* __restrict__ keys, u32 npush, u32* __restrict__ pool, PushSeg* __restrict__ segs, u32 seg_cap,
                                 LevelScalars* __restrict__ sc) {
    const u32 i = blockIdx.x * blockDim.x + threadIdx.x;
    if (i >= npush) return;
    const u32 tgt = (u32)(keys[i] >> 32);
    pool[i] = (u32)keys[i];
    if (i == 0 || (u32)(keys[i - 1] >> 32) != tgt) {
        const u32 j = atomicAdd(&sc->nseg, 1u);
        if (j < SEG_INLINE) sc->segs[j] = PushSeg{tgt, i};
        if (j < seg_cap) segs[j] = PushSeg{tgt, i};
    }
}

__global__ __launch_bounds__(256) void live_max_level_kernel(const u32* __restrict__ levels, const u32* __restrict__ pos, size_t lo, size_t hi,
                                                              const u32* __restrict__ cur, u32* __restrict__ d_max) {
    u32 best = 0;
    const size_t stride = (size_t)gridDim.x * blockDim.x;
    for (size_t k = lo + (size_t)blockIdx.x * blockDim.x + threadIdx.x; k < hi; k += stride) {
        const u32 lv = levels[k];
        if (lv > best && cur[pos[k]] == lv) best = lv;
    }
    best = wave_reduce_max(best);
// ... 299 lines not shown
```

### tudocomp_amd/csrc/factorize_tiles.hip

```cpp
#include "stages.hpp"
#include "prim.hpp"
#include "factorize_tiles.hpp"

#include <stdlib.h>

namespace tdc {

namespace {

#ifndef TDC_WIN_TW
#define TDC_WIN_TW 16384
#endif
#ifndef TDC_WIN_WPE
#define TDC_WIN_WPE 7
#endif
#ifndef TDC_WIN_LB
#define TDC_WIN_LB 4
#endif
#ifndef TDC_WIN_TE
#define TDC_WIN_TE 512
#endif
#ifndef TDC_WIN_TT
#define TDC_WIN_TT 256
#endif
constexpr int TW = TDC_WIN_TW;
constexpr int TH_MAX = 2048;
constexpr int TT = TDC_WIN_TT;
constexpr int TCH = 64;
constexpr int TE_SMALL = TDC_WIN_TE;
constexpr int TE_LARGE = 8192;
#ifndef TDC_WIN_TT_LARGE
#define TDC_WIN_TT_LARGE 1024
#endif
constexpr int TT_LARGE = TDC_WIN_TT_LARGE;

__device__ __forceinline__ int PA(int q) {
    const int t = q >> 6, w = (q >> 2) & 15;
    return (t << 6) + (((w + 2 * (t >> 2)) & 15) << 2) + (q & 3);
}
__device__ __forceinline__ int PW(int t, int k) { return (t << 6) + (((2 * k + 2 * (t >> 2)) & 15) << 2); }
constexpr int BIG = 1 << 29;

enum : u32 { B_VAL = 0x3Fu, B_START = 0x40u, B_TRUNC = 0x80u };
__device__ __forceinline__ u32 b_ub(u32 b) { return (b & B_START) ? 0u : (b & B_VAL); }

enum : u32 { S_UND = 0, S_SEL = 1, S_REJ = 2, S_UNC = 3 };
__device__ __forceinline__ int e_pos(u32 e) { return (int)(e & 0xFFFFu); }
__device__ __forceinline__ u32 e_state(u32 e) { return (e >> 16) & 3u; }
__device__ __forceinline__ u32 e_trunc(u32 e) { return (e >> 18) & 1u; }
__device__ __forceinline__ void e_set_state(u32* ent, int i, u32 e, u32 st) { lds_store(&ent[i], (e & ~(3u << 16)) | (st << 16)); }

struct WinScalars { u32 fail; int min_margin; unsigned long long factors; u32 max_entries, pad; unsigned long long prof[16]; };

#ifdef TDC_WIN_PROF
#define WPROF_DECL unsigned long long wp_t = __builtin_readcyclecounter(); unsigned long long wp_acc[12] = {0,0,0,0,0,0,0,0,0,0,0,0};
#define WPROF(i) do { const unsigned long long wp_n = __builtin_readcyclecounter(); wp_acc[i] += wp_n - wp_t; wp_t = wp_n; } while (0)
#define WPROF_CNT(i, v) do { wp_acc[i] += (v); } while (0)
#define WPROF_FLUSH do { if (tid == 0) for (int wi = 0; wi < 12; ++wi) atomicAdd(&sc->prof[wi], wp_acc[wi]); } while (0)
#define WTRIP(i) do { if (tid < 64) { const u64 wt_a = __ballot(true); if (lane == __builtin_ctzll(wt_a)) atomicAdd(&sc->prof[i], 1ull); } } while (0)
#else
#define WPROF_DECL
#define WPROF(i) do {} while (0)
#define WPROF_CNT(i, v) do {} while (0)
#define WPROF_FLUSH do {} while (0)
#define WTRIP(i) do {} while (0)
#endif

__device__ __forceinline__ void lds_barrier() { asm volatile("s_waitcnt lgkmcnt(0)\n\ts_barrier" ::: "memory"); }

__device__ __forceinline__ u32 hit4(u32 w, u32 pat) {
    const u32 x = (w & 0x7F7F7F7Fu) ^ pat;
    return ~(x + 0x7F7F7F7Fu) & 0x80808080u;
}
template <int KT, int TE, int WPE, int WSRC>
__global__ __launch_bounds__(KT) __attribute__((amdgpu_waves_per_eu(WPE, WPE))) void window_eager_kernel(const u32* __restrict__ cur_g, const u32* __restrict__ prio_g,
                                                            const u8* __restrict__ res_g, const u32* __restrict__ phi, size_t n,
                                                            u32 lcut, u32 threshold, u32 ntiles, u32 halo,
                                                            u32* __restrict__ flen, u8* __restrict__ flen8, u32* __restrict__ fsrc, WinScalars* __restrict__ sc) {
    constexpr int NWV = KT / 64;
    constexpr int CPT = TW / (64 * KT) > 0 ? TW / (64 * KT) : 1;
    static_assert(TW % 64 == 0 && TW / 64 <= KT * CPT, "every chunk of the window needs an owner");
    static_assert(TW <= 65536, "16-bit window positions");
    __shared__ __attribute__((aligned(16))) u8 S[TW];
    __shared__ u32 ent[TE];
    __shared__ u32 pri[TE];
    __shared__ unsigned short selp[NWV][64];
    __shared__ u32 wtot[NWV];
    __shared__ int s_und[3];
    __shared__ int s_tl, s_tr;
    __shared__ u64 s_lvlmask;
    const int tid = threadIdx.x;
    const int lane = tid & 63, wv = tid >> 6;
    WPROF_DECL

    const size_t TH = halo, TI = (size_t)TW - 2 * (size_t)halo;
    for (u32 tile = blockIdx.x; tile < ntiles; tile += gridDim.x) {
        const size_t a = (size_t)tile * TI;
        const size_t b = (a + TI < n) ? a + TI : n;
        const size_t w0 = (a >= (size_t)TH) ? a - TH : 0;
        const size_t w1 = (b + TH < n) ? b + TH : n;
        const int wl = (int)(w1 - w0);
        const int ia = (int)(a - w0), ib = (int)(b - w0);
        const int mid = wl / 2;
        __syncthreads();
        WPROF(0);
        if (tid == 0) { s_und[0] = 0; s_und[1] = 0; s_und[2] = 0; s_tl = -BIG; s_tr = BIG; s_lvlmask = 0; }
        __syncthreads();
        u64 mymask = 0;
        constexpr int LIT = TW / (KT * 4);
        constexpr int LB = LIT < TDC_WIN_LB ? LIT : TDC_WIN_LB;
        static_assert(TW % (KT * 4) == 0 && LIT % LB == 0, "window load");
        if (wl == TW) {
#pragma unroll 1
            for (int it0 = 0; it0 < LIT; it0 += LB) {
                uint4 cv[LB];
                u32 rv4[LB];
                u64 bmask = 0;
#pragma unroll
                for (int u = 0; u < LB; ++u) {
                    const size_t gp = w0 + (size_t)((it0 + u) * KT * 4 + tid * 4);
                    cv[u] = *(const uint4*)(cur_g + gp);
                    rv4[u] = *(const u32*)(res_g + gp);
                }
#pragma unroll
                for (int u = 0; u < LB; ++u) {
                    const int i = (it0 + u) * KT * 4 + tid * 4;
                    const u32 c4[4] = { cv[u].x, cv[u].y, cv[u].z, cv[u].w };
                    u32 sw = 0;
#pragma unroll
                    for (int k = 0; k < 4; ++k) {
                        u32 c = c4[k] > 63u ? 63u : c4[k];
                        if (c < threshold) c = 0;
                        const u32 rv = (rv4[u] >> (8 * k)) & 0xFFu;
                        const u32 bb = c ? (c | (rv != c ? B_TRUNC : 0u)) : 0u;
                        sw |= bb << (8 * k);
                        bmask |= 1ull << c;
                    }
                    *(u32*)&S[PA(i)] = sw;
                }
                mymask |= bmask;
            }
        } else {
            for (int i = tid * 4; i < TW; i += KT * 4) {
                u32 sw = 0;
                const size_t gp = w0 + i;
                if (gp + 4 <= w1) {
                    const uint4 cv = *(const uint4*)(cur_g + gp);
                    const u32 rv4 = *(const u32*)(res_g + gp);
                    const u32 c4[4] = { cv.x, cv.y, cv.z, cv.w };
#pragma unroll
                    for (int k = 0; k < 4; ++k) {
                        u32 c = c4[k] > 63u ? 63u : c4[k];
                        if (c < threshold) c = 0;
                        const u32 rv = (rv4 >> (8 * k)) & 0xFFu;
                        const u32 bb = c ? (c | (rv != c ? B_TRUNC : 0u)) : 0u;
                        sw |= bb << (8 * k);
                        mymask |= 1ull << c;
                    }
                } else {
#pragma unroll
                    for (int k = 0; k < 4; ++k) {
// ... 168 lines not shown
                    const int i = i0 + lane * NWV + wv;
                    const bool have = i < m;
                    const u32 e = have ? lds_load(&ent[i]) : 0u;
                    const u32 s = have ? e_state(e) : (u32)S_REJ;
                    const int p = e_pos(e);
                    if (pass == 0 && s == S_UNC) {
                        if (p < mid) atomicMax(&s_tl, p + iL); else atomicMin(&s_tr, p - (iL - 1));
                    }
                    const u64 selm = __ballot(s == S_SEL);
                    if (!selm) continue;
                    const int nsel = (int)__popcll(selm);
                    if (s == S_SEL) lds_store(&selp[wv][__popcll(selm & ((1ull << lane) - 1ull))], (unsigned short)p);
                    __builtin_amdgcn_wave_barrier();
                    for (int b0 = 0; b0 < nsel; b0 += EPB) {
                        WTRIP(15);
                        const int k = b0 + gi;
                        if (k < nsel && gj < iL) {
                            const int ps = (int)lds_load(&selp[wv][k]);
                            if (pass == 0) {
                                const int d = gj + 1, q = ps - d;
                                if (d < iL && q >= 0) {
                                    const u32 bb = S[PA(q)];
                                    if (!(bb & B_START) && (bb & B_VAL) > (u32)d) {
                                        const bool alive = (u32)d >= threshold;
                                        S[PA(q)] = alive ? (u8)(B_TRUNC | (u32)d) : (u8)0;
                                        if (alive) newlv |= 1ull << d;
                                    }
                                }
                            } else {
                                const int q = ps + gj;
                                if (q < wl) S[PA(q)] = (gj == 0) ? (u8)(B_START | L) : (u8)0;
                            }
                        }
                    }
                    __builtin_amdgcn_wave_barrier();
                }
                if (pass == 0) {
                    newlv &= ~lvl_seen;
#pragma unroll
                    for (int d = 32; d >= 1; d >>= 1) newlv |= __shfl_xor(newlv, d, 64);
                    if (lane == 0 && newlv) atomicOr((unsigned long long*)&s_lvlmask, (unsigned long long)newlv);
                    lds_barrier();
                }
            }
            lds_barrier();
            WPROF(5);
            int nfl = dfl, nfr = dfr;
            const int tl = lds_load(&s_tl), tr = lds_load(&s_tr);
            if (tl > nfl) nfl = tl;
            if (tr < nfr) nfr = tr;
            fl = nfl; fr = nfr;
            if (tl > -BIG || tr < BIG) {
                lds_barrier();
                if (tid == 0) { s_tl = -BIG; s_tr = BIG; }
            }
            WPROF(6);
        }
        if (tid == 0 && !failed) {
            int mg = BIG;
            if (fl > -BIG / 2) mg = ia - fl;
            if (fr < BIG / 2 && fr - ib < mg) mg = fr - ib;
            atomicMin(&sc->min_margin, mg);
        }
        if (failed || fl > ia || fr < ib) { if (tid == 0) atomicOr(&sc->fail, failed ? 2u : 1u); }
        else {
#pragma unroll
            for (int cc = 0; cc < CPT; ++cc) {
                const int chunk = tid * CPT + cc;
                const int base = chunk * TCH;
                if (base < TW && base < ib && base + TCH > ia) {
#pragma unroll
                    for (int k = 0; k < TCH; k += 8) {
                        const u64 rw = *(const u64*)&S[PW(chunk, k >> 3)];
                        u64 w = rw & 0x4040404040404040ull;
                        while (w) {
                            const int bb = __builtin_ctzll(w) >> 3;
                            w &= w - 1;
                            const int pos = base + k + bb;
                            if (pos < ia || pos >= ib) continue;
                            const size_t gp = w0 + pos;
                            if (flen8) flen8[gp] = (u8)((rw >> (8 * bb)) & 0x3Fu);
                            else flen[gp] = (u32)(rw >> (8 * bb)) & 0x3Fu;
                            if constexpr (WSRC == 1) fsrc[gp] = phi[gp];
                            else if constexpr (WSRC == 2) { const u32 r = prio_g[gp]; if (r < (u32)n) fsrc[gp] = r ? phi[r - 1] : phi[n - 1]; }
                            ++nsel_interior;
                        }
                    }
                }
            }
        }
        nsel_interior = wave_reduce_sum(nsel_interior);
        if (lane == 0 && nsel_interior) atomicAdd(&sc->factors, (unsigned long long)nsel_interior);
        WPROF(7);
    }
    WPROF_FLUSH;
}

__global__ void window_cleanup_kernel(u32* __restrict__ flen, u8* __restrict__ flen8, size_t n, u32 lcut) {
    const size_t p = (size_t)blockIdx.x * blockDim.x + threadIdx.x;
    if (p >= n) return;
    if (flen8) { if (flen8[p] <= lcut) flen8[p] = 0; }
    else if (flen[p] <= lcut) flen[p] = 0;
}

}

u32 window_levels_max_lcut() { return 63; }
u32 window_levels_window() { return (u32)TW; }
u32 window_levels_small_list() { return (u32)TE_SMALL; }
size_t window_levels_min_text() { return (size_t)4 * TW; }

int factorize_window_levels(Ctx& c, size_t n, const u32* cur, const u32* prio, const u8* res8, const u32* phi, u32 lcut, u32 threshold,
                            FactorSpace fs, u64* nfactors, bool start_large, const u32* src_sa) {
    *nfactors = 0;
    if (lcut < threshold) return 0;
    hipStream_t s = c.stream;
    const size_t mark = c.arena.mark();
    u32 halo = (u32)c.window_halo & ~3u;
    if (halo < 2 * lcut + 64) halo = (2 * lcut + 64 + 3) & ~3u;
    if (halo > (u32)TH_MAX) halo = TH_MAX;
    bool large = c.window_large_lists != 0 || start_large;
    const u32 max_grid = 1u << 20;
    WinScalars* d_sc = (WinScalars*)c.arena.alloc(sizeof(WinScalars));
    WinScalars h;
    int result = 0;
    for (int attempt = 0; attempt < 4; ++attempt) {
        const size_t ti = (size_t)TW - 2 * (size_t)halo;
        const u32 ntiles = cdiv(n, ti);
        const u32 grid = ntiles < max_grid ? ntiles : max_grid;
        HIP_TRY(hipMemsetAsync(d_sc, 0, sizeof(WinScalars), s));
        HIP_TRY(hipMemsetD32Async((hipDeviceptr_t)&d_sc->min_margin, BIG, 1, s));
        {
            Ctx::ProfScope prof(c, K_WINDOW_LEVELS, (u64)((double)n * TW / ti * 5) + (u64)n * 2);
            if (!large) {
                if (phi) window_eager_kernel<TT, TE_SMALL, TDC_WIN_WPE, 1><<<grid, TT, 0, s>>>(cur, prio, res8, phi, n, lcut, threshold, ntiles, halo, fs.flen, fs.flen8, fs.fsrc, d_sc);
                else if (src_sa) window_eager_kernel<TT, TE_SMALL, TDC_WIN_WPE, 2><<<grid, TT, 0, s>>>(cur, prio, res8, src_sa, n, lcut, threshold, ntiles, halo, fs.flen, fs.flen8, fs.fsrc, d_sc);
                else window_eager_kernel<TT, TE_SMALL, TDC_WIN_WPE, 0><<<grid, TT, 0, s>>>(cur, prio, res8, phi, n, lcut, threshold, ntiles, halo, fs.flen, fs.flen8, fs.fsrc, d_sc);
            } else {
                if (phi) window_eager_kernel<TT_LARGE, TE_LARGE, TT_LARGE / 256, 1><<<grid, TT_LARGE, 0, s>>>(cur, prio, res8, phi, n, lcut, threshold, ntiles, halo, fs.flen, fs.flen8, fs.fsrc, d_sc);
                else if (src_sa) window_eager_kernel<TT_LARGE, TE_LARGE, TT_LARGE / 256, 2><<<grid, TT_LARGE, 0, s>>>(cur, prio, res8, src_sa, n, lcut, threshold, ntiles, halo, fs.flen, fs.flen8, fs.fsrc, d_sc);
                else window_eager_kernel<TT_LARGE, TE_LARGE, TT_LARGE / 256, 0><<<grid, TT_LARGE, 0, s>>>(cur, prio, res8, phi, n, lcut, threshold, ntiles, halo, fs.flen, fs.flen8, fs.fsrc, d_sc);
            }
            LAUNCH_CHECK();
        }
        h = c.read(d_sc);
#ifdef TDC_WIN_PROF
        {
            static const char* nm[16] = { "wait_prev", "load", "dense", "scan+write", "select", "apply", "borders", "tail", "levels", "entries", "rounds", "w0 collect3+", "w0 round body", "w0 walk left", "w0 walk right", "w0 apply batch" };
            for (int i = 0; i < 16; ++i) fprintf(stderr, "winprof %-10s %llu\n", nm[i], h.prof[i]);
            fprintf(stderr, "winprof windows %u grid %u attempt %d halo %u min_margin %d fail %u max_entries %u\n", ntiles, grid, attempt,
                    halo, h.min_margin, h.fail, h.max_entries);
        }
#endif
        if (c.level_log) fprintf(stderr, "window pass: attempt %d halo %u lists %s -> fail %u, smallest margin %d\n", attempt, halo, large ? "large" : "small", h.fail, h.min_margin);
        if (c.window_force_fail) h.fail |= 1u;
        result = (int)h.fail;
        if (!h.fail) break;
        window_cleanup_kernel<<<cdiv(n, 256), 256, 0, s>>>(fs.flen, fs.flen8, n, lcut);
        LAUNCH_CHECK();
        bool again = false;
        if ((h.fail & 2u) && !large) { large = true; again = true; }
        if ((h.fail & 1u) && halo < (u32)TH_MAX && !c.window_force_fail) { halo = TH_MAX; again = true; }
        if (!again) break;
    }
    c.arena.release(mark);
    if (result == 0) *nfactors = h.factors;
    return result;
}

}
```

### tudocomp_amd/csrc/factorize_tiles.hpp

```cpp
#pragma once
#include "stages.hpp"

namespace tdc {

int factorize_window_levels(Ctx& c, size_t n, const u32* cur, const u32* prio, const u8* res8, const u32* phi, u32 lcut, u32 threshold,
                             FactorSpace fs, u64* nfactors, bool start_large = false, const u32* src_sa = nullptr);
u32 window_levels_window();
u32 window_levels_small_list();
u32 window_levels_max_lcut();
size_t window_levels_min_text();

}
```

### tudocomp_amd/csrc/flatten.hip

```cpp
#include "stages.hpp"
#include "prim.hpp"

#include <stdlib.h>

namespace tdc {

__global__ void fstart_flag_kernel(const u32* __restrict__ flen, const u32* __restrict__ owner, size_t n, u32* __restrict__ flag) {
    const size_t p = (size_t)blockIdx.x * blockDim.x + threadIdx.x;
    if (p >= n) return;
    const u32 o = owner[p];
    flag[p] = (flen[p] != 0 && o != NONE32 && (p == 0 || owner[p - 1] != o)) ? 1u : 0u;
}
__global__ void fstart_scatter_kernel(const u32* __restrict__ flen, const u32* __restrict__ owner, const u32* __restrict__ fsrc,
                                      const u32* __restrict__ offs, size_t n, size_t cap, u32* __restrict__ pos,
                                      u32* __restrict__ src, u32* __restrict__ len) {
    const size_t p = (size_t)blockIdx.x * blockDim.x + threadIdx.x;
    if (p >= n) return;
    const u32 l = flen[p];
    const u32 ow = owner[p];
    if (l != 0 && ow != NONE32 && (p == 0 || owner[p - 1] != ow)) {
        const u32 o = offs[p];
        if (o < cap) {
            pos[o] = (u32)p;
            if (src) src[o] = fsrc[p];
            if (len) len[o] = l;
        }
    }
}

size_t extract_factors(Ctx& c, size_t n, FactorSpace fs, u32* pos, u32* src, u32* len, size_t cap) {
    if (n == 0) return 0;
    if (fs.owner_rem_bits) throw HipError{hipErrorUnknown, "extract_factors: owner[] carries remainder bits", (int)__LINE__};
    const size_t mark = c.arena.mark();
    u32* offs = c.arena.get<u32>(n);
    u32* d_total = c.arena.get<u32>(1);
    const unsigned gn = cdiv(n, 256);
    {
        Ctx::ProfScope prof(c, K_EXTRACT, (u64)n * 12);
        fstart_flag_kernel<<<gn, 256, 0, c.stream>>>(fs.flen, fs.owner, n, offs);
        LAUNCH_CHECK();
    }
    exclusive_sum_u32(c, offs, offs, n, d_total);
    {
        Ctx::ProfScope prof(c, K_EXTRACT, (u64)n * 12);
        fstart_scatter_kernel<<<gn, 256, 0, c.stream>>>(fs.flen, fs.owner, fs.fsrc, offs, n, cap, pos, src, len);
        LAUNCH_CHECK();
    }
    const size_t z = c.read(d_total);
    c.arena.release(mark);
    return z;
}

constexpr int OW_T = 256, OW_PER = 16, OW_TILE = OW_T * OW_PER;
__host__ __device__ __forceinline__ u32 owner_rem_bits_for(u32 z, u32 cap) {
    u32 b = 0;
    while (b < cap && (((u64)z + 1) >> (31 - b)) == 0) ++b;
    return b;
}
__device__ __forceinline__ u32 ow_idx(u32 i) { return i + (i >> 4); }

__global__ __launch_bounds__(OW_T) void owner_count_kernel(const u32* __restrict__ flen, const u8* __restrict__ flen8, size_t n, u32* __restrict__ tilecnt) {
    __shared__ u32 sm[OW_T / 64];
    const size_t base = (size_t)blockIdx.x * OW_TILE;
    u32 cnt = 0;
    if (flen8) {
        const size_t p = base + (size_t)threadIdx.x * OW_PER;
        if (p + OW_PER <= n) {
            const uint4 v = *(const uint4*)(flen8 + p);
            const u32 w4[4] = { v.x, v.y, v.z, v.w };
#pragma unroll
            for (int k = 0; k < 4; ++k) {
                const u32 w = w4[k];
                const u32 nz = ((w & 0x7F7F7F7Fu) + 0x7F7F7F7Fu) | w;
                cnt += (u32)__popc(nz & 0x80808080u);
            }
        } else {
            for (int k = 0; k < OW_PER; ++k) if (p + k < n && flen8[p + k] != 0) ++cnt;
        }
    } else {
#pragma unroll
        for (int r = 0; r < OW_PER / 4; ++r) {
            const size_t p = base + ((size_t)r * OW_T + threadIdx.x) * 4;
            if (p + 4 <= n) {
                const uint4 v = *(const uint4*)(flen + p);
                cnt += (v.x != 0) + (v.y != 0) + (v.z != 0) + (v.w != 0);
            } else {
                for (int k = 0; k < 4; ++k) if (p + k < n && flen[p + k] != 0) ++cnt;
            }
        }
    }
    cnt = wave_reduce_sum(cnt);
    if (lane_id() == 0) sm[wave_id()] = cnt;
    __syncthreads();
    if (threadIdx.x == 0) { u32 t = 0; for (int i = 0; i < OW_T / 64; ++i) t += sm[i]; tilecnt[blockIdx.x] = t; }
}

__global__ __launch_bounds__(OW_T) void owner_build_kernel(const u32* __restrict__ flen, const u8* __restrict__ flen8, size_t n, const u32* __restrict__ tilebase,
                                                           u32* __restrict__ pos, u32* __restrict__ owner, uint2* __restrict__ cross,
                                                           u8* __restrict__ cls, u32* __restrict__ lenl, const u32* __restrict__ rem_total, u32 rem_cap) {
    __shared__ u32 s[OW_TILE + OW_TILE / 16 + 16];
    __shared__ u32 sm[OW_T / 64 + 1], smx[OW_T / 64];
    const size_t base = (size_t)blockIdx.x * OW_TILE;
    const int lane = lane_id(), w = wave_id();
    if (flen8) {
        const u32 i = threadIdx.x * OW_PER;
        const size_t p = base + i;
        u32 w4[4] = { 0, 0, 0, 0 };
        if (p + OW_PER <= n) { const uint4 v = *(const uint4*)(flen8 + p); w4[0] = v.x; w4[1] = v.y; w4[2] = v.z; w4[3] = v.w; }
        else for (int k = 0; k < OW_PER; ++k) if (p + k < n) w4[k >> 2] |= (u32)flen8[p + k] << (8 * (k & 3));
#pragma unroll
        for (int k = 0; k < OW_PER; ++k) {
            u32 l = (w4[k >> 2] >> (8 * (k & 3))) & 0xFFu;
            if (l == 255u) l = flen[p + k];
            s[ow_idx(i + k)] = l;
        }
    } else {
#pragma unroll
    for (int r = 0; r < OW_PER / 4; ++r) {
        const u32 i = ((u32)r * OW_T + threadIdx.x) * 4;
        const size_t p = base + i;
        uint4 v = make_uint4(0, 0, 0, 0);
        if (p + 4 <= n) v = *(const uint4*)(flen + p);
        else {
            if (p < n) v.x = flen[p];
            if (p + 1 < n) v.y = flen[p + 1];
            if (p + 2 < n) v.z = flen[p + 2];
        }
        const u32 q = ow_idx(i);
        s[q] = v.x; s[q + 1] = v.y; s[q + 2] = v.z; s[q + 3] = v.w;
    }
    }
    __syncthreads();
    const u32 l0 = threadIdx.x * OW_PER;
    u32 f[OW_PER];
    u32 cnt = 0, mylast = 0;
#pragma unroll
    for (int k = 0; k < OW_PER; ++k) {
        f[k] = s[ow_idx(l0 + k)];
        if (f[k] != 0) { ++cnt; mylast = l0 + k + 1; }
    }
    u32 total;
    const u32 excl = block_exclusive_sum<u32, OW_T / 64>(cnt, sm, total);
    const u32 inc = wave_inclusive_max(mylast);
    if (lane == 63) smx[w] = inc;
    __syncthreads();
    u32 cur_start = __shfl_up(inc, 1, 64);
    if (lane == 0) cur_start = 0;
    for (int i = 0; i < w; ++i) cur_start = max(cur_start, smx[i]);
    u32 rank = tilebase[blockIdx.x] + excl;
    u32 cur_rank = rank - 1;
    u32 cur_len = cur_start ? s[ow_idx(cur_start - 1)] : 0u;
    u32 out[OW_PER];
    const bool stage_starts = total <= (u32)OW_TILE / 2;
    const u32 remb = rem_total ? owner_rem_bits_for(*rem_total, rem_cap) : 0u;
    const u32 qmax = (1u << remb) - 1u, rsh = (32u - remb) & 31u;
#pragma unroll
    for (int k = 0; k < OW_PER; ++k) {
        const u32 pl = l0 + k;
        if (f[k] != 0) {
            cur_start = pl + 1; cur_len = f[k]; cur_rank = rank++;
            if (!stage_starts && base + pl < n) { pos[cur_rank] = (u32)(base + pl); if (lenl) lenl[cur_rank] = f[k]; }
        }
        const u32 d = pl - (cur_start - 1);
        out[k] = (cur_start != 0 && d < cur_len) ? (cur_rank | (min(cur_len - d - 1u, qmax) << rsh)) : NONE32;
    }
    if (cls) {
        u32 w4[4] = { 0, 0, 0, 0 };
#pragma unroll
        for (int k = 0; k < OW_PER; ++k) {
            const u32 cl = (out[k] == NONE32) ? 0u : (f[k] != 0 ? 2u : 3u);
            w4[k >> 2] |= cl << (8 * (k & 3));
        }
        const size_t p = base + l0;
        if (p + OW_PER <= n) *(uint4*)(cls + p) = make_uint4(w4[0], w4[1], w4[2], w4[3]);
        else for (int k = 0; k < OW_PER; ++k) if (p + k < n) cls[p + k] = (u8)(w4[k >> 2] >> (8 * (k & 3)));
    }
    if (threadIdx.x == OW_T - 1) {
        const u32 end = cur_start ? cur_start - 1 + cur_len : 0u;
        cross[blockIdx.x] = (end > (u32)OW_TILE) ? make_uint2(cur_rank, end - (u32)OW_TILE) : make_uint2(NONE32, 0u);
    }
    __syncthreads();
#pragma unroll
    for (int k = 0; k < OW_PER; ++k) s[ow_idx(l0 + k)] = out[k];
    __syncthreads();
#pragma unroll
    for (int r = 0; r < OW_PER / 4; ++r) {
        const u32 i = ((u32)r * OW_T + threadIdx.x) * 4;
        const size_t p = base + i;
        const u32 q = ow_idx(i);
        if (p + 4 <= n) *(uint4*)(owner + p) = make_uint4(s[q], s[q + 1], s[q + 2], s[q + 3]);
        else for (int k = 0; k < 4; ++k) if (p + k < n) owner[p + k] = s[q + k];
    }
    if (stage_starts && total) {
        __syncthreads();
        u32 o = excl;
#pragma unroll
        for (int k = 0; k < OW_PER; ++k) if (f[k] != 0) { s[o] = l0 + k; s[OW_TILE / 2 + o] = f[k]; ++o; }
        __syncthreads();
        const u32 tb = tilebase[blockIdx.x];
        for (u32 e = threadIdx.x; e < total; e += OW_T) {
            const size_t p = base + s[e];
            if (p < n) { pos[tb + e] = (u32)p; if (lenl) lenl[tb + e] = s[OW_TILE / 2 + e]; }
        }
    }
}

__global__ __launch_bounds__(256) void owner_cross_kernel(const uint2* __restrict__ cross, size_t n, u32* __restrict__ owner, u8* __restrict__ cls,
                                                          const u32* __restrict__ rem_total, u32 rem_cap) {
    const uint2 cr = cross[blockIdx.x];
    if (cr.y == 0) return;
    const u32 remb = rem_total ? owner_rem_bits_for(*rem_total, rem_cap) : 0u;
    const u32 qmax = (1u << remb) - 1u, rsh = (32u - remb) & 31u;
    const size_t start = ((size_t)blockIdx.x + 1) * OW_TILE;
    for (size_t j = threadIdx.x; j < cr.y && start + j < n; j += 256) {
        owner[start + j] = cr.x | (min(cr.y - (u32)j - 1u, qmax) << rsh);
        if (cls) cls[start + j] = (u8)3;
    }
}

void build_owner(Ctx& c, size_t n, FactorSpace& fs) {
    fs.have_list = false;
    fs.have_cls = false;
    fs.owner_rem_bits = 0;
    if (n == 0) return;
    const size_t mark = c.arena.mark();
    const u32 tiles = cdiv(n, OW_TILE);
    u32* tilecnt = c.arena.get<u32>(tiles);
    uint2* cross = (uint2*)c.arena.alloc((size_t)tiles * sizeof(uint2));
    u32* pos = fs.fpos ? fs.fpos : c.arena.get<u32>(n);
    u32* d_total = c.arena.get<u32>(1);
    {
        Ctx::ProfScope prof(c, K_EXTRACT, (u64)n * (fs.flen8 ? 1 : 4));
        owner_count_kernel<<<tiles, OW_T, 0, c.stream>>>(fs.flen, fs.flen8, n, tilecnt);
        LAUNCH_CHECK();
    }
    exclusive_sum_u32(c, tilecnt, tilecnt, tiles, d_total);
    {
        Ctx::ProfScope prof(c, K_EXTRACT, (u64)n * (fs.flen8 ? 6 : 9));
        const u32* rem_total = fs.want_owner_rem ? d_total : nullptr;
        const u32 rem_cap = std::min<u32>(fs.want_owner_rem, 8u);
        owner_build_kernel<<<tiles, OW_T, 0, c.stream>>>(fs.flen, fs.flen8, n, tilecnt, pos, fs.owner, cross, fs.cls, fs.fpos ? fs.flenl : nullptr, rem_total, rem_cap);
        LAUNCH_CHECK();
        owner_cross_kernel<<<tiles, 256, 0, c.stream>>>(cross, n, fs.owner, fs.cls, rem_total, rem_cap);
        fs.have_cls = fs.cls != nullptr;
        LAUNCH_CHECK();
    }
    const size_t z = c.read(d_total);
    if (fs.fpos) { fs.nfact = z; fs.have_list = true; }
    fs.owner_rem_bits = fs.want_owner_rem ? owner_rem_bits_for((u32)z, std::min<u32>(fs.want_owner_rem, 8u)) : 0u;
    c.arena.release(mark);
}

__global__ void expand_flen8_kernel(const u8* __restrict__ flen8, size_t n, u32* __restrict__ flen) {
    const size_t p = (size_t)blockIdx.x * blockDim.x + threadIdx.x;
    if (p >= n) return;
    const u32 l = flen8[p];
    if (l != 255u) flen[p] = l;
}
void expand_flen8(Ctx& c, size_t n, FactorSpace& fs) {
    if (!fs.flen8) return;
    if (n) { expand_flen8_kernel<<<cdiv(n, 256), 256, 0, c.stream>>>(fs.flen8, n, fs.flen); LAUNCH_CHECK(); }
    fs.flen8 = nullptr;
}

__global__ void fspace_clear_kernel(size_t n, u32* __restrict__ flen, u32* __restrict__ owner) {
    const size_t p = (size_t)blockIdx.x * blockDim.x + threadIdx.x;
    if (p >= n) return;
    flen[p] = 0;
    owner[p] = NONE32;
}
__global__ void fspace_scatter_kernel(const u32* __restrict__ pos, const u32* __restrict__ src, const u32* __restrict__ len,
                                      size_t z, size_t n, u32* __restrict__ flen, u32* __restrict__ owner, u32* __restrict__ fsrc) {
    const size_t i = (size_t)blockIdx.x * blockDim.x + threadIdx.x;
    if (i >= z) return;
    const u32 p = pos[i], l = len[i];
    if ((size_t)p + l > n) return;
    flen[p] = l;
    fsrc[p] = src[i];
    for (u32 j = 0; j < l; ++j) owner[p + j] = (u32)i;
}

void scatter_factors(Ctx& c, size_t n, const u32* pos, const u32* src, const u32* len, size_t z, FactorSpace fs) {
    if (n == 0) return;
    fspace_clear_kernel<<<cdiv(n, 256), 256, 0, c.stream>>>(n, fs.flen, fs.owner);
    LAUNCH_CHECK();
    if (z) {
        fspace_scatter_kernel<<<cdiv(z, 256), 256, 0, c.stream>>>(pos, src, len, z, n, fs.flen, fs.owner, fs.fsrc);
        LAUNCH_CHECK();
    }
}

constexpr u32 NOT_DONE = 0xFFFFFFFFu;

struct FlattenScalars { u32 waiting; u32 num_flattened; u32 max_depth; u32 pad; unsigned long long steps, waits; };

__device__ __forceinline__ u32 lazy_source(const u32* __restrict__ prio, const u32* __restrict__ sa, size_t n, const u32* __restrict__ fsrc, u32 p) {
    const u32 r = prio[p];
    return r < (u32)n ? (r ? sa[r - 1] : sa[n - 1]) : fsrc[p];
}
__global__ void flatten_init_kernel(const u32* __restrict__ fpos, size_t z, const u32* __restrict__ flen, const u32* __restrict__ orig,
                                    uint4* __restrict__ rec, const u32* __restrict__ lenl, const u32* __restrict__ src_prio,
                                    const u32* __restrict__ src_sa, size_t src_n) {
    const size_t i = (size_t)blockIdx.x * blockDim.x + threadIdx.x;
    if (i >= z) return;
    const u32 p = fpos[i];
    const u32 o = src_prio ? lazy_source(src_prio, src_sa, src_n, orig, p) : orig[p];
    rec[i] = make_uint4(p, lenl ? lenl[i] : flen[p], o, NOT_DONE);
}
__global__ void sources_fill_kernel(const u32* __restrict__ fpos, size_t z, const u32* __restrict__ src_prio, const u32* __restrict__ src_sa,
                                    size_t src_n, u32* fsrc) {
    const size_t i = (size_t)blockIdx.x * blockDim.x + threadIdx.x;
    if (i >= z) return;
    const u32 p = fpos[i];
    fsrc[p] = lazy_source(src_prio, src_sa, src_n, fsrc, p);
}
__global__ void sources_fill_pos_kernel(const u32* __restrict__ flen, size_t n, const u32* __restrict__ src_prio, const u32* __restrict__ src_sa,
                                        size_t src_n, u32* fsrc) {
    const size_t p = (size_t)blockIdx.x * blockDim.x + threadIdx.x;
    if (p < n && flen[p]) fsrc[p] = lazy_source(src_prio, src_sa, src_n, fsrc, (u32)p);
}

#ifndef TDC_FL_K
#define TDC_FL_K 4
#endif
constexpr int FL_K = TDC_FL_K;
template <bool FIRST, bool REM>
__global__ __launch_bounds__(256) void flatten_round_kernel(const uint4* __restrict__ work, u32 nwork, size_t n, const u32* __restrict__ owner,
                                                             uint4* rec, uint4* __restrict__ next, FlattenScalars* __restrict__ sc, u32 max_steps, u32 rem_bits, u32 first) {
    const u32 rsh = 32u - rem_bits, qmax = (1u << rem_bits) - 1u, rmask = REM ? ((1u << rsh) - 1u) : 0xFFFFFFFFu;
    __shared__ u32 sm[5];
    __shared__ u32 s_base;
    const u32 base = blockIdx.x * (256u * FL_K);
    u32 fi[FL_K], len[FL_K], src[FL_K], dep[FL_K];
    u32 act = 0, fin = 0, valid = 0;
#pragma unroll
    for (int r = 0; r < FL_K; ++r) {
        const u32 j = base + (u32)r * 256u + threadIdx.x;
        fi[r] = 0; len[r] = 0; src[r] = 0; dep[r] = 0;
        if (j < nwork) {
            if (FIRST) { const uint4 me = rec[first + j]; fi[r] = first + j; len[r] = me.y; src[r] = me.z; }
            else { const uint4 it = work[j]; fi[r] = it.x; len[r] = it.y; src[r] = it.z; dep[r] = it.w; }
            valid |= 1u << r;
        }
    }
    act = valid;
#ifdef TDC_FL_PROF
    u32 psteps = 0, pwaits = 0;
#endif
    for (u32 step = 0; step < max_steps && __any(act != 0); ++step) {
        u32 rr[FL_K];
#pragma unroll
        for (int r = 0; r < FL_K; ++r) {
            rr[r] = NONE32;
            if (act & (1u << r)) {
                if ((size_t)src[r] >= n || dep[r] >= n) { act &= ~(1u << r); fin |= 1u << r; }
                else rr[r] = owner[src[r]];
            }
        }
#ifdef TDC_FL_PROF
        psteps += (u32)__popc(act);
#endif
        uint4 sr[FL_K];
#pragma unroll
        for (int r = 0; r < FL_K; ++r) {
            sr[r] = make_uint4(0, 0, 0, 0);
            if (act & (1u << r)) {
                if (rr[r] == NONE32) { act &= ~(1u << r); fin |= 1u << r; }
                else {
                    if (REM) {
                        const u32 q = rr[r] >> rsh;
                        rr[r] &= rmask;
                        if (q < qmax && len[r] > q + 1u) { act &= ~(1u << r); fin |= 1u << r; continue; }
                    }
                    sr[r] = rec[rr[r]];
                }
            }
        }
#pragma unroll
        for (int r = 0; r < FL_K; ++r) {
            if (!(act & (1u << r))) continue;
            const u32 d = src[r] - sr[r].x;
            if ((u64)d + len[r] > sr[r].y) { act &= ~(1u << r); fin |= 1u << r; continue; }
            u32 ssrc;
            if (rr[r] < fi[r]) {
                ssrc = sr[r].w;
                if (ssrc == NOT_DONE) { act &= ~(1u << r);
#ifdef TDC_FL_PROF
                    ++pwaits;
#endif
                    continue; }
            } else {
                ssrc = sr[r].z;
            }
            src[r] = ssrc + d;
            ++dep[r];
        }
    }
#ifdef TDC_FL_PROF
    { const u32 a = wave_reduce_sum(psteps), b = wave_reduce_sum(pwaits);
      if (lane_id() == 0) { atomicAdd(&sc->steps, (unsigned long long)a); atomicAdd(&sc->waits, (unsigned long long)b); } }
#endif
    u32 nflat = 0, mxdep = 0;
#pragma unroll
    for (int r = 0; r < FL_K; ++r) {
        if (fin & (1u << r)) {
            ((u32*)&rec[fi[r]])[3] = src[r];
            if (dep[r]) { ++nflat; mxdep = max(mxdep, dep[r]); }
        }
    }
    const u32 wmask = valid & ~fin;
    u32 total;
    u32 off = block_exclusive_sum<u32, 4>((u32)__popc(wmask), sm, total);
    if (threadIdx.x == 0) s_base = total ? atomicAdd(&sc->waiting, total) : 0u;
    __syncthreads();
    off += s_base;
#pragma unroll
    for (int r = 0; r < FL_K; ++r)
        if (wmask & (1u << r)) next[off++] = make_uint4(fi[r], len[r], src[r], dep[r]);
    nflat = wave_reduce_sum(nflat);
    mxdep = wave_reduce_max(mxdep);
    if (lane_id() == 0 && nflat) { atomicAdd(&sc->num_flattened, nflat); atomicMax(&sc->max_depth, mxdep); }
}

__global__ void flatten_commit_kernel(size_t z, const uint4* __restrict__ rec, u32* __restrict__ fsrc) {
    const size_t i = (size_t)blockIdx.x * blockDim.x + threadIdx.x;
    if (i >= z) return;
    const uint4 q = rec[i];
    if (q.w != q.z) fsrc[q.x] = q.w;
}

void materialize_sources(Ctx& c, size_t n, FactorSpace& fs) {
    if (!fs.src_prio) return;
    if (n) {
        if (fs.have_list) { if (fs.nfact) sources_fill_kernel<<<cdiv(fs.nfact, 256), 256, 0, c.stream>>>(fs.fpos, fs.nfact, fs.src_prio, fs.src_sa, fs.src_n, fs.fsrc); }
        else sources_fill_pos_kernel<<<cdiv(n, 256), 256, 0, c.stream>>>(fs.flen, n, fs.src_prio, fs.src_sa, fs.src_n, fs.fsrc);
        LAUNCH_CHECK();
    }
    fs.src_prio = nullptr;
}

void flatten_factors(Ctx& c, size_t n, FactorSpace fs, FlattenStats* st, const std::function<void(int)>& between, void* rec_keep,
                     u32 chunks, const std::function<void(u32, size_t)>& chunk_done) {
    if (fs.src_prio && !rec_keep) materialize_sources(c, n, fs);
    FlattenStats local;
    if (!st) st = &local;
    *st = FlattenStats();
    if (n == 0) { if (between) between(0); return; }
    hipStream_t s = c.stream;
    const size_t mark = c.arena.mark();
    u32* fpos = fs.have_list ? fs.fpos : c.arena.get<u32>(n);
    const size_t z = fs.have_list ? fs.nfact : extract_factors(c, n, fs, fpos, nullptr, nullptr, n);
    if (z == 0) { if (between) between(0); c.arena.release(mark); return; }
    const u32 K = flatten_chunk_count(chunks ? chunks : (u32)c.flatten_chunks, z);
    uint4* rec = rec_keep ? (uint4*)rec_keep : (uint4*)c.arena.alloc(z * sizeof(uint4));
    FlattenScalars* d_sc = (FlattenScalars*)c.arena.alloc(sizeof(FlattenScalars));
    HIP_TRY(hipMemsetAsync(d_sc, 0, sizeof(FlattenScalars), s));
    const unsigned gz = cdiv(z, 256);
    flatten_init_kernel<<<gz, 256, 0, s>>>(fpos, z, fs.flen, fs.fsrc, rec, fs.have_list ? fs.flenl : nullptr, fs.src_prio, fs.src_sa, fs.src_n);
    LAUNCH_CHECK();
    const size_t cmax = (z + K - 1) / K;
    uint4* work[2] = { (uint4*)c.arena.alloc(cmax * sizeof(uint4)), nullptr };
    u32 flat_growth = (u32)c.flatten_growth;
    if (flat_growth < 2) flat_growth = 2;
    for (u32 k = 0; k < K; ++k) {
        const size_t r0 = flatten_chunk_start(z, k, K), r1 = flatten_chunk_start(z, k + 1, K);
        u32 waiting = (u32)(r1 - r0);
        int cur_w = -1;
        u32 max_steps = (u32)c.flatten_steps;
        if (max_steps == 0) max_steps = 1u << 30;
        u32 stalled = 0;
        while (waiting) {
            const int nxt = cur_w < 0 ? 0 : (cur_w ^ 1);
            if (!work[nxt]) work[nxt] = (uint4*)c.arena.alloc((K == 1 ? (size_t)waiting : cmax) * sizeof(uint4));
            HIP_TRY(hipMemsetAsync(&d_sc->waiting, 0, sizeof(u32), s));
            {
                Ctx::ProfScope prof(c, K_FLATTEN_ROUND, (u64)waiting * 52);
                const u32 rb = fs.owner_rem_bits;
                const unsigned g = cdiv(waiting, 256 * FL_K);
                if (cur_w < 0) { if (rb) flatten_round_kernel<true, true><<<g, 256, 0, s>>>(nullptr, waiting, n, fs.owner, rec, work[nxt], d_sc, max_steps, rb, (u32)r0);
                                 else flatten_round_kernel<true, false><<<g, 256, 0, s>>>(nullptr, waiting, n, fs.owner, rec, work[nxt], d_sc, max_steps, 0u, (u32)r0); }
                else { if (rb) flatten_round_kernel<false, true><<<g, 256, 0, s>>>(work[cur_w], waiting, n, fs.owner, rec, work[nxt], d_sc, max_steps, rb, 0u);
                       else flatten_round_kernel<false, false><<<g, 256, 0, s>>>(work[cur_w], waiting, n, fs.owner, rec, work[nxt], d_sc, max_steps, 0u, 0u); }
                LAUNCH_CHECK();
            }
            if (between) between((int)st->rounds + 1);
            const u32 now = c.read(&d_sc->waiting);
            st->rounds++;
            if (c.level_log) {
                const FlattenScalars hs = c.read(d_sc);
                fprintf(stderr, "flatten round %u (range %u of %u): %u waiting -> %u (budget %u steps; cumulative: %llu visits, %llu of them waits)\n", st->rounds, k + 1, K, waiting, now, max_steps, hs.steps, hs.waits);
            }
            stalled = (now == waiting) ? stalled + 1 : 0;
            if (now > waiting || (now == waiting && max_steps >= (1u << 30)) || stalled > 40)
                throw HipError{hipErrorUnknown, "flatten: rounds made no progress", (int)__LINE__};
            waiting = now;
            cur_w = nxt;
            if (max_steps < (1u << 30)) max_steps = (max_steps > (1u << 30) / flat_growth) ? (1u << 30) : max_steps * flat_growth;
        }
        if (chunk_done) chunk_done(k, r1);
    }
    if (between) between(0);
    if (!rec_keep) {
        flatten_commit_kernel<<<gz, 256, 0, s>>>(z, rec, fs.fsrc);
        LAUNCH_CHECK();
    }
    FlattenScalars h = c.read(d_sc);
    st->num_flattened = h.num_flattened;
    st->max_depth_lb = h.max_depth;
    c.arena.release(mark);
}

}
```

### tudocomp_amd/csrc/stages.hpp

```cpp
#pragma once
#include "common.hpp"
#include <functional>

namespace tdc {

size_t escape_device(Ctx& c, const u8* d_in, size_t n, u8* d_out);
size_t count_escapes_device(Ctx& c, const u8* d_in, size_t n);

struct SAStats { u32 rounds = 0; u32 sym_bits = 0; u32 init_syms = 0; u64 sorted_elems = 0;
                 u32 wide_kw = 0;  u32 text_rounds = 0; u64 wide_nonheads = 0;
                 u32 overlapped = 0;
                 u64 pair_resolved = 0;
                 u64 star_chains = 0;  };
struct SAExtra { u8* lcp8 = nullptr; int mode = 0; };

void build_suffix_array(Ctx& c, const u8* text, size_t n, u32* sa, u32* isa, SAStats* st, SAExtra* ex = nullptr);
struct CandFused {
    u32 threshold = 0, lcut = 0;
    u8* cls = nullptr;
    u8* res8 = nullptr;
    u8* flen8 = nullptr;
    u32* flen = nullptr;
    u32* tilecnt = nullptr;
    u32* acc = nullptr;
    u32* lvlhist = nullptr;
    u32* entries = nullptr;
    bool filled = false;
};
constexpr u32 CF_COPIES = 64, CF_ACC = 80;
void build_isa_phi_plcp_fused(Ctx& c, const u32* sa, const u8* lcp8, size_t n, u32* isa, u32* phi, u32* plcp, u32* d_maxlcp, CandFused* cf = nullptr);
bool fused_scatter_has_image(const Ctx& c, size_t n);
u32 factorize_arrays_lcut0(const Ctx& c, size_t n, u32 threshold);
void text_histogram_add(Ctx& c, const u8* part, size_t len, u32* d_hist);
void text_histogram_finish(Ctx& c, const u8* text, size_t n, const u32* d_hist);

void build_phi(Ctx& c, const u32* sa, size_t n, u32* phi);
void build_plcp(Ctx& c, const u8* text, size_t n, const u32* phi, u32* plcp, u32* d_maxlcp);
void build_lce_with_carry(Ctx& c, const u8* text, size_t n, const u32* src, u32* len, u32* d_max);
void build_lcp(Ctx& c, const u32* sa, const u32* plcp, size_t n, u32* lcp);

struct FactorSpace {
    u32* flen = nullptr;
    u8* flen8 = nullptr;
    u32* owner = nullptr;
    u32* fsrc = nullptr;
    u32* fpos = nullptr;
    u32* flenl = nullptr;
    size_t nfact = 0;
    bool have_list = false;
    u8* cls = nullptr;
    bool have_cls = false;
    u32 want_owner_rem = 0;
    u32 owner_rem_bits = 0;
    const u32* src_prio = nullptr;
    const u32* src_sa = nullptr;
    size_t src_n = 0;
};
inline const u32* plain_owner(const FactorSpace& fs) {
    if (fs.owner_rem_bits) throw HipError{hipErrorUnknown, "owner[] carries remainder bits (FactorSpace::owner_rem_bits): this stage reads plain ranks", (int)__LINE__};
    return fs.owner;
}
void materialize_sources(Ctx& c, size_t n, FactorSpace& fs);

struct FactorizeStats { u64 factors = 0; u32 maxlcp = 0; u32 levels = 0; u32 rounds = 0; u64 pushes = 0; u64 entries = 0; u32 small_levels = 0; u32 purges = 0;
                        u32 window_pass = 0;
                        u32 window_lcut = 0;
                        u32 probes = 0;
                        u32 max_push_targets = 0;
                        u32 eager_levels = 0, eager_phases = 0;  };

void factorize_arrays(Ctx& c, size_t n, const u32* sa, u32* isa, const u32* phi, u32* plcp, u32 maxlcp,
                      u32 threshold, FactorSpace& fs, FactorizeStats* st, const CandFused* cf = nullptr);

void build_owner(Ctx& c, size_t n, FactorSpace& fs);
void expand_flen8(Ctx& c, size_t n, FactorSpace& fs);

void plcp_peaks_factorize(Ctx& c, size_t n, const u32* phi, const u32* plcp, u32 threshold, FactorSpace& fs, u64* nfactors);
void factorize_max_lcp(Ctx& c, size_t n, u32* isa, const u32* phi, u32* plcp, u32 maxlcp, u32 threshold, FactorSpace& fs,
                       FactorizeStats* st);

void factorize_max_heap(Ctx& c, size_t n, const u32* sa, const u32* isa, const u32* plcp, u32 maxlcp, u32 threshold, FactorSpace& fs,
                        FactorizeStats* st);

struct FlattenStats { u64 num_flattened = 0; u64 max_depth_lb = 0; u32 rounds = 0; };
constexpr u32 FLATTEN_MAX_CHUNKS = 16;
inline u32 flatten_chunk_count(u32 want, size_t z) { return (u32)std::max<size_t>(1, std::min<size_t>(std::min<size_t>(want, FLATTEN_MAX_CHUNKS), z)); }
inline size_t flatten_chunk_start(size_t z, u32 k, u32 K) { return (size_t)((u64)z * k / K); }
void flatten_factors(Ctx& c, size_t n, FactorSpace fs, FlattenStats* st, const std::function<void(int)>& between = {}, void* rec_keep = nullptr,
                     u32 chunks = 0, const std::function<void(u32, size_t)>& chunk_done = {});

size_t extract_factors(Ctx& c, size_t n, FactorSpace fs, u32* pos, u32* src, u32* len, size_t cap);
void scatter_factors(Ctx& c, size_t n, const u32* pos, const u32* src, const u32* len, size_t z, FactorSpace fs);

struct EncodeStats { u64 factors = 0; u64 flen_min = 0, flen_max = 0, fdist_max = 0; u64 out_bits = 0; u32 sigma = 0; };
size_t encode_huff(Ctx& c, const u8* text, size_t n, FactorSpace fs, u8* d_out, size_t out_cap, EncodeStats* st);
struct EncodeEarly;
size_t encode_stream(Ctx& c, const u8* text, size_t n, FactorSpace fs, int coder, u8* d_out, size_t out_cap, EncodeStats* st, EncodeEarly* early = nullptr);
EncodeEarly* encode_early_reserve(Ctx& c, size_t n, size_t z_rec = 0);
void* encode_early_rec(EncodeEarly* e);
void encode_early_run(Ctx& c, const u8* text, size_t n, FactorSpace fs, int coder, EncodeEarly* e, bool finish = true);
void encode_early_free(EncodeEarly* e);
bool encode_early_chunks(Ctx& c, size_t n, const FactorSpace& fs, EncodeEarly* e, u32 K, size_t out_cap);
void encode_early_chunk_done(Ctx& c, const u8* text, size_t n, const FactorSpace& fs, EncodeEarly* e, u32 k);
u8* encode_early_out(EncodeEarly* e, size_t* out_cap);
u32 encode_early_packed(const EncodeEarly* e);

size_t encode_bound(size_t n);
size_t encode_bound_coder(size_t n, int coder);
size_t encode_bound_uni(size_t n, int coder);

struct LzssStats { u64 factors = 0; };
void lzss_lcp_factorize(Ctx& c, const u8* text, size_t n, const u32* sa, const u32* isa, u32 threshold, FactorSpace fs,
                        LzssStats* st);

}
#include <vector>
namespace tdc {
struct DecodeStats { u64 factors = 0; u32 rounds = 0; u32 device_parse = 0; };
struct StreamFormatError { const char* what; };
struct Sink {
    u8* into = nullptr; size_t cap = 0;
    u8* owned = nullptr;
    uint8_t** out = nullptr; size_t* out_len = nullptr;
    bool keep = false;
    Sink() = default;
    Sink(Sink&& o) : into(o.into), cap(o.cap), owned(o.owned), out(o.out), out_len(o.out_len), keep(o.keep) { o.owned = nullptr; }
    Sink(const Sink&) = delete;
    Sink& operator=(const Sink&) = delete;
    ~Sink() { free(owned); }
    u8* release() { u8* r = owned; owned = nullptr; return r; }
};
size_t decode_lzss(Ctx& c, const u8* stream, size_t len, int coder, Sink& out, DecodeStats* st);
bool decode_lzss_uni(Ctx& c, const u8* stream, size_t len, int kind, Sink& out, DecodeStats* st, size_t* n_out);
struct DecodeTooLarge { u64 n; };
size_t decode_lz78_gamma(Ctx& c, const u8* stream, size_t len, Sink& out, size_t* need, DecodeStats* st);
size_t lz78_parse_host(const u8* in, size_t n, std::vector<u32>& ids, std::vector<u8>& chars, bool* leftover_is_high);
size_t lz78_gamma_encode(Ctx& c, const u32* d_ids, const u8* d_chars, size_t z, u8* d_out, size_t out_cap);
size_t gamma_encode_items(Ctx& c, const u32* d_ids, const u8* d_chars, size_t z, u8* d_out, size_t out_cap);

size_t lzw_parse_host(const u8* in, size_t n, std::vector<u32>& codes);
size_t lzw_encode(Ctx& c, const u32* d_codes, size_t z, bool bit, u8* d_out, size_t out_cap);
constexpr size_t LZW_DEVICE_MIN = (size_t)64 << 10;
size_t decode_lzw(Ctx& c, const u8* stream, size_t len, bool bit, Sink& out, size_t* need, DecodeStats* st);

constexpr u32 LZSS_SW_MAX_WINDOW = 4096;
size_t lzss_sw_tokens(Ctx& c, const u8* d_text, size_t n, u32 window, u32 threshold, u32** tokpos, u32** fac);
size_t lzss_sw_factor_list(Ctx& c, const u32* tokpos, const u32* fac, size_t ntok, u32* d_pos, u32* d_src, u32* d_len);
struct LzssSwStats { u64 factors = 0; u32 flen_max = 0; bool truncates = false; };
size_t lzss_sw_encode_tokens(Ctx& c, const u8* d_text, const u32* tokpos, const u32* fac, size_t ntok, u32 window, int kind,
                             u8* d_out, size_t out_cap, LzssSwStats* st);
size_t lzss_sw_bound(size_t n, u32 window, int kind);
bool decode_lzss_sw(Ctx& c, const u8* stream, size_t len, int kind, u32 window, Sink& out, size_t* need, DecodeStats* st, size_t* n_out);
int lzss_sw_decode_host(const u8* in, size_t len, int coder, u32 window, std::vector<u8>& text);

struct LzssSwBatch {
    const u32* off = nullptr;
    u64* gfirst = nullptr;
    u64* ooff = nullptr;
    u32* flag = nullptr;
    size_t ntok = 0; u64 factors = 0;
    const u32* tokpos = nullptr, *fac = nullptr; const u64* gpos = nullptr;
};
void lzss_sw_batch_sizes(Ctx& c, const u8* d_text, size_t n, size_t count, u32 window, u32 threshold, int kind, LzssSwBatch& B);
void lzss_sw_batch_pack(Ctx& c, const u8* d_text, size_t count, u32 window, int kind, const LzssSwBatch& B, u8* d_out, size_t used);
struct LzssSwBatchDec {
    const u8* blob = nullptr; u64 sub = 0;
    const u64* s_off = nullptr, *s_len = nullptr;
    u32* tlen = nullptr; int* status = nullptr; u64* ooff = nullptr; u64* factors = nullptr;
};
void lzss_sw_batch_decode_sizes(Ctx& c, int kind, u32 window, size_t count, LzssSwBatchDec& D);
void lzss_sw_batch_decode_write(Ctx& c, int kind, u32 window, size_t count, const LzssSwBatchDec& D, u8* d_text);

struct LzBatchDec {
    const u8* blob = nullptr; u64 sub = 0;
    const u64* s_off = nullptr, *s_len = nullptr;
    u64* bits = nullptr;
    int* status = nullptr;
    u64* item_off = nullptr;
    u64* ooff = nullptr;
    u64* factors = nullptr;
};
// ... 26 lines not shown
```

Before: 8904 MB/s.

## Build flatten records in owner kernel and store window sources half-indexed

The owner-build kernel now writes the flatten records (pos, len, source, NOT_DONE) directly into the arena slot the early encoder will reuse, so flatten can skip its separate init kernel and the extra pass over fpos/flenl/fsrc. The window factorization kernel can also write sources for short factors into a half-sized array indexed by p>>1, which avoids scattered writes into the full fsrc array. This adds an earlier host read of the factor count, a conditional rec allocation, and several arena-placement sanity checks that throw if the layout assumptions break.

```diff
diff --git a/include/tdc_gpu.h b/include/tdc_gpu.h
--- a/include/tdc_gpu.h
+++ b/include/tdc_gpu.h
@@ -70,7 +70,7 @@
     uint32_t tie_rounds;
     uint32_t rebuilds;
     float ms_round_first, ms_round_last, ms_round_tie;
-    float reserved1;
+    uint32_t records_from_build;
 } tdc_gpu_stats;
 
 int  tdc_gpu_ctx_create(int device, tdc_gpu_ctx** ctx);
diff --git a/tudocomp_amd/_native.py b/tudocomp_amd/_native.py
--- a/tudocomp_amd/_native.py
+++ b/tudocomp_amd/_native.py
@@ -53,7 +53,7 @@
         [("pipe_stages", ctypes.c_uint32), ("pipe_dev", ctypes.c_uint32), ("pipe_len", ctypes.c_uint64 * 8), ("pipe_ms", ctypes.c_float * 8),
          ("ranges_early", ctypes.c_uint32), ("len_rounds", ctypes.c_uint32),
          ("rules", ctypes.c_uint64), ("replaced", ctypes.c_uint64), ("tie_rounds", ctypes.c_uint32), ("rebuilds", ctypes.c_uint32),
-         ("ms_round_first", ctypes.c_float), ("ms_round_last", ctypes.c_float), ("ms_round_tie", ctypes.c_float), ("reserved1", ctypes.c_float)])
+         ("ms_round_first", ctypes.c_float), ("ms_round_last", ctypes.c_float), ("ms_round_tie", ctypes.c_float), ("records_from_build", ctypes.c_uint32)])
 
     def as_dict(self):
         d = {k: getattr(self, k) for k, _ in self._fields_}
diff --git a/tudocomp_amd/csrc/api_compress.hip b/tudocomp_amd/csrc/api_compress.hip
--- a/tudocomp_amd/csrc/api_compress.hip
+++ b/tudocomp_amd/csrc/api_compress.hip
@@ -87,6 +87,9 @@
     const bool early_planned = early_is_planned(c, n, threshold, flatten, strategy, enc_coder, d_text);
     if (early_planned && c.flen_bytes && !A.fs.flen8) A.fs.flen8 = c.arena.get<u8>(n + 64);
     A.fs.want_owner_rem = early_planned ? (u32)c.owner_rem : 0u;
+    const bool rec_path = early_planned && A.fs.flen8 && !A.phi;
+    A.fs.want_rec = rec_path && c.owner_rec;
+    A.fs.want_half = rec_path && c.src_half;
     FactorizeStats fz;
     FlattenStats fl;
     const int e0 = ev ? ev->tick() : 0;
@@ -98,8 +101,11 @@
     const bool early = flatten && enc_coder == 0 && d_text && c.enc_early && c.huff_ok && n >= (c.enc_early >= 2 ? (size_t)1 : ((size_t)1 << 20)) &&
                        A.fs.have_list && A.fs.have_cls && A.fs.flenl && A.fs.nfact > 0;
     if (!early) expand_flen8(c, n, A.fs);
+    if (A.fs.nfact == 0) A.fs.half = nullptr;
+    if (A.fs.half && !(early && c.enc_rec))
+        throw HipError{hipErrorUnknown, "factorize: half-indexed sources on a path that does not keep the flatten records", (int)__LINE__};
     if (early) {
-        A.early = encode_early_reserve(c, n, c.enc_rec ? A.fs.nfact : 0);
+        A.early = encode_early_reserve(c, n, c.enc_rec ? A.fs.nfact : 0, c.enc_rec ? A.fs.rec : nullptr);
         u32 K = c.flatten_chunks ? (u32)c.flatten_chunks : (u32)std::min<size_t>(A.fs.nfact / FLAT_CHUNK_MIN, FLAT_CHUNK_MAX);
         K = flatten_chunk_count(K, A.fs.nfact);
         const bool packed = K >= 2 && encode_early_chunks(c, n, A.fs, A.early, K, align_up(encode_bound_coder(n, enc_coder) + 16, 8));
@@ -123,6 +129,7 @@
         st->probes = fz.probes; st->max_push_targets = fz.max_push_targets;
         st->num_flattened = fl.num_flattened; st->max_depth_lb = fl.max_depth_lb; st->flatten_rounds = fl.rounds;
         st->ranges_early = A.early ? encode_early_packed(A.early) : 0u;
+        st->records_from_build = fl.rec_from_build ? 1u : 0u;
         if (ev) { ev->span(&st->ms_factorize, e0, e1); ev->span(&st->ms_flatten, e1, e2); }
     }
 }
diff --git a/tudocomp_amd/csrc/api_ctx.hip b/tudocomp_amd/csrc/api_ctx.hip
--- a/tudocomp_amd/csrc/api_ctx.hip
+++ b/tudocomp_amd/csrc/api_ctx.hip
@@ -131,7 +131,9 @@
 const OptionDef FOLD_OPTIONS[] = {
     { "fused_cand",       [](Ctx& c, long v) { c.fused_cand = v != 0; } },
     { "sel_tile_counts",  [](Ctx& c, long v) { c.sel_tile_counts = v != 0; } },
-    { "flatten_chunks",   [](Ctx& c, long v) { c.flatten_chunks = clampi(v, 0, (long)FLATTEN_MAX_CHUNKS); } },
+    { "owner_rec",        [](Ctx& c, long v) { c.owner_rec = v != 0; } },
+    { "src_half",         [](Ctx& c, long v) { c.src_half = v != 0; } },
+    { "flatten_chunks",  [](Ctx& c, long v) { c.flatten_chunks = clampi(v, 0, (long)FLATTEN_MAX_CHUNKS); } },
     { "repair_recount",   [](Ctx& c, long v) { c.repair_recount = v != 0; } },
     { "repair_table_bits",[](Ctx& c, long v) { c.repair_table_bits = v == 0 ? 0 : clampi(v, 8, 30); } },
     { "repair_log",       [](Ctx& c, long v) { c.repair_log = v != 0; } },
diff --git a/tudocomp_amd/csrc/common.hpp b/tudocomp_amd/csrc/common.hpp
--- a/tudocomp_amd/csrc/common.hpp
+++ b/tudocomp_amd/csrc/common.hpp
@@ -140,6 +140,8 @@
     int enc_early = 1;
     int fused_cand = 1;
     int sel_tile_counts = 1;
+    int owner_rec = 1;
+    int src_half = 1;
     int fs_pair = 1;
     int small_big = 1;
     int small_pipeline = 1;
diff --git a/tudocomp_amd/csrc/encode.hip b/tudocomp_amd/csrc/encode.hip
--- a/tudocomp_amd/csrc/encode.hip
+++ b/tudocomp_amd/csrc/encode.hip
@@ -604,9 +604,12 @@
     } while (finish && E.step < 3);
 }
 
-EncodeEarly* encode_early_reserve(Ctx& c, size_t n, size_t z_rec) {
+EncodeEarly* encode_early_reserve(Ctx& c, size_t n, size_t z_rec, const void* rec_placed) {
     EncodeEarly* E = new EncodeEarly();
-    try { encode_reserve(c, n, *E, z_rec); } catch (...) { delete E; throw; }
+    try {
+        encode_reserve(c, n, *E, z_rec);
+        if (rec_placed && E->rec != rec_placed) throw HipError{hipErrorUnknown, "encode: the records of build_owner are not where this reservation puts them", (int)__LINE__};
+    } catch (...) { delete E; throw; }
     return E;
 }
 void* encode_early_rec(EncodeEarly* E) { return E->rec; }
diff --git a/tudocomp_amd/csrc/factorize.hip b/tudocomp_amd/csrc/factorize.hip
--- a/tudocomp_amd/csrc/factorize.hip
+++ b/tudocomp_amd/csrc/factorize.hip
@@ -975,7 +975,8 @@
                                                                     phi ? nullptr : sa, isa, fs.fsrc, fs.flen8);
         LAUNCH_CHECK();
     }
-    if ((u64)maxlcp + 1 <= threshold || threshold == 0) { c.arena.release(mark); build_owner(c, n, fs); if (!phi) { fs.src_prio = prio; fs.src_sa = sa; fs.src_n = n; } return; }
+    fs.half = nullptr;
+    if ((u64)maxlcp + 1 <= threshold || threshold == 0) { c.arena.release(mark); fs.want_rec = false; build_owner(c, n, fs); if (!phi) { fs.src_prio = prio; fs.src_sa = sa; fs.src_n = n; } return; }
     const size_t nlev = (size_t)maxlcp + 2;
     u64* rkey = c.arena.get<u64>(n + 2);
     u32* d_segstart = (u32*)rkey;
@@ -1202,9 +1203,11 @@
                 start_large = (double)mx * 16.0 * (double)window_levels_window() / (double)n > 4.0 * (double)window_levels_small_list();
             }
             const bool wsrc = !phi && c.window_src;
-            const int why = factorize_window_levels(c, n, cur, prio, res8, phi, lcut, threshold, fs, &nf, start_large, wsrc ? sa : nullptr);
+            u32* half = wsrc && fs.want_half && threshold >= 2 ? (u32*)skeys[1] : nullptr;
+            const int why = factorize_window_levels(c, n, cur, prio, res8, phi, lcut, threshold, fs, &nf, start_large, wsrc ? sa : nullptr, half);
             const bool ok = why == 0;
             if (ok && wsrc) window_src_done = true;
+            if (ok && half) { fs.half = half; fs.half_lcut = lcut; }
             st->window_pass = ok ? 1 : 2;
             st->window_lcut = lcut;
             if (ok) { st->factors += nf; break; }
@@ -1687,6 +1690,7 @@
         }
     }
     c.arena.release(mark);
+    if (!window_src_done) fs.want_rec = false;
     build_owner(c, n, fs); if (!phi && !window_src_done) { fs.src_prio = prio; fs.src_sa = sa; fs.src_n = n; }
 }
 
diff --git a/tudocomp_amd/csrc/factorize_tiles.hip b/tudocomp_amd/csrc/factorize_tiles.hip
--- a/tudocomp_amd/csrc/factorize_tiles.hip
+++ b/tudocomp_amd/csrc/factorize_tiles.hip
@@ -76,7 +76,8 @@
 __global__ __launch_bounds__(KT) __attribute__((amdgpu_waves_per_eu(WPE, WPE))) void window_eager_kernel(const u32* __restrict__ cur_g, const u32* __restrict__ prio_g,
                                                             const u8* __restrict__ res_g, const u32* __restrict__ phi, size_t n,
                                                             u32 lcut, u32 threshold, u32 ntiles, u32 halo,
-                                                            u32* __restrict__ flen, u8* __restrict__ flen8, u32* __restrict__ fsrc, WinScalars* __restrict__ sc) {
+                                                            u32* __restrict__ flen, u8* __restrict__ flen8, u32* __restrict__ fsrc, u32* __restrict__ half,
+                                                            WinScalars* __restrict__ sc) {
     constexpr int NWV = KT / 64;
     constexpr int CPT = TW / (64 * KT) > 0 ? TW / (64 * KT) : 1;
     static_assert(TW % 64 == 0 && TW / 64 <= KT * CPT, "every chunk of the window needs an owner");
@@ -411,7 +412,11 @@
                             if (flen8) flen8[gp] = (u8)((rw >> (8 * bb)) & 0x3Fu);
                             else flen[gp] = (u32)(rw >> (8 * bb)) & 0x3Fu;
                             if constexpr (WSRC == 1) fsrc[gp] = phi[gp];
-                            else if constexpr (WSRC == 2) { const u32 r = prio_g[gp]; if (r < (u32)n) fsrc[gp] = r ? phi[r - 1] : phi[n - 1]; }
+                            else if constexpr (WSRC == 2) {
+                                const u32 r = prio_g[gp];
+                                if (half) half[gp >> 1] = r < (u32)n ? (r ? phi[r - 1] : phi[n - 1]) : fsrc[gp];
+                                else if (r < (u32)n) fsrc[gp] = r ? phi[r - 1] : phi[n - 1];
+                            }
                             ++nsel_interior;
                         }
                     }
@@ -440,7 +445,7 @@
 size_t window_levels_min_text() { return (size_t)4 * TW; }
 
 int factorize_window_levels(Ctx& c, size_t n, const u32* cur, const u32* prio, const u8* res8, const u32* phi, u32 lcut, u32 threshold,
-                            FactorSpace fs, u64* nfactors, bool start_large, const u32* src_sa) {
+                            FactorSpace fs, u64* nfactors, bool start_large, const u32* src_sa, u32* half) {
     *nfactors = 0;
     if (lcut < threshold) return 0;
     hipStream_t s = c.stream;
@@ -462,13 +467,13 @@
         {
             Ctx::ProfScope prof(c, K_WINDOW_LEVELS, (u64)((double)n * TW / ti * 5) + (u64)n * 2);
             if (!large) {
-                if (phi) window_eager_kernel<TT, TE_SMALL, TDC_WIN_WPE, 1><<<grid, TT, 0, s>>>(cur, prio, res8, phi, n, lcut, threshold, ntiles, halo, fs.flen, fs.flen8, fs.fsrc, d_sc);
-                else if (src_sa) window_eager_kernel<TT, TE_SMALL, TDC_WIN_WPE, 2><<<grid, TT, 0, s>>>(cur, prio, res8, src_sa, n, lcut, threshold, ntiles, halo, fs.flen, fs.flen8, fs.fsrc, d_sc);
-                else window_eager_kernel<TT, TE_SMALL, TDC_WIN_WPE, 0><<<grid, TT, 0, s>>>(cur, prio, res8, phi, n, lcut, threshold, ntiles, halo, fs.flen, fs.flen8, fs.fsrc, d_sc);
+                if (phi) window_eager_kernel<TT, TE_SMALL, TDC_WIN_WPE, 1><<<grid, TT, 0, s>>>(cur, prio, res8, phi, n, lcut, threshold, ntiles, halo, fs.flen, fs.flen8, fs.fsrc, half, d_sc);
+                else if (src_sa) window_eager_kernel<TT, TE_SMALL, TDC_WIN_WPE, 2><<<grid, TT, 0, s>>>(cur, prio, res8, src_sa, n, lcut, threshold, ntiles, halo, fs.flen, fs.flen8, fs.fsrc, half, d_sc);
+                else window_eager_kernel<TT, TE_SMALL, TDC_WIN_WPE, 0><<<grid, TT, 0, s>>>(cur, prio, res8, phi, n, lcut, threshold, ntiles, halo, fs.flen, fs.flen8, fs.fsrc, half, d_sc);
             } else {
-                if (phi) window_eager_kernel<TT_LARGE, TE_LARGE, TT_LARGE / 256, 1><<<grid, TT_LARGE, 0, s>>>(cur, prio, res8, phi, n, lcut, threshold, ntiles, halo, fs.flen, fs.flen8, fs.fsrc, d_sc);
-                else if (src_sa) window_eager_kernel<TT_LARGE, TE_LARGE, TT_LARGE / 256, 2><<<grid, TT_LARGE, 0, s>>>(cur, prio, res8, src_sa, n, lcut, threshold, ntiles, halo, fs.flen, fs.flen8, fs.fsrc, d_sc);
-                else window_eager_kernel<TT_LARGE, TE_LARGE, TT_LARGE / 256, 0><<<grid, TT_LARGE, 0, s>>>(cur, prio, res8, phi, n, lcut, threshold, ntiles, halo, fs.flen, fs.flen8, fs.fsrc, d_sc);
+                if (phi) window_eager_kernel<TT_LARGE, TE_LARGE, TT_LARGE / 256, 1><<<grid, TT_LARGE, 0, s>>>(cur, prio, res8, phi, n, lcut, threshold, ntiles, halo, fs.flen, fs.flen8, fs.fsrc, half, d_sc);
+                else if (src_sa) window_eager_kernel<TT_LARGE, TE_LARGE, TT_LARGE / 256, 2><<<grid, TT_LARGE, 0, s>>>(cur, prio, res8, src_sa, n, lcut, threshold, ntiles, halo, fs.flen, fs.flen8, fs.fsrc, half, d_sc);
+                else window_eager_kernel<TT_LARGE, TE_LARGE, TT_LARGE / 256, 0><<<grid, TT_LARGE, 0, s>>>(cur, prio, res8, phi, n, lcut, threshold, ntiles, halo, fs.flen, fs.flen8, fs.fsrc, half, d_sc);
             }
             LAUNCH_CHECK();
         }
diff --git a/tudocomp_amd/csrc/factorize_tiles.hpp b/tudocomp_amd/csrc/factorize_tiles.hpp
--- a/tudocomp_amd/csrc/factorize_tiles.hpp
+++ b/tudocomp_amd/csrc/factorize_tiles.hpp
@@ -4,7 +4,8 @@
 namespace tdc {
 
 int factorize_window_levels(Ctx& c, size_t n, const u32* cur, const u32* prio, const u8* res8, const u32* phi, u32 lcut, u32 threshold,
-                             FactorSpace fs, u64* nfactors, bool start_large = false, const u32* src_sa = nullptr);
+                             FactorSpace fs, u64* nfactors, bool start_large = false, const u32* src_sa = nullptr,
+                             u32* half = nullptr);
 u32 window_levels_window();
 u32 window_levels_small_list();
 u32 window_levels_max_lcut();
diff --git a/tudocomp_amd/csrc/flatten.hip b/tudocomp_amd/csrc/flatten.hip
--- a/tudocomp_amd/csrc/flatten.hip
+++ b/tudocomp_amd/csrc/flatten.hip
@@ -52,6 +52,10 @@
 }
 
 constexpr int OW_T = 256, OW_PER = 16, OW_TILE = OW_T * OW_PER;
+constexpr u32 NOT_DONE = 0xFFFFFFFFu;
+__device__ __forceinline__ u32 factor_source(const u32* __restrict__ fsrc, const u32* __restrict__ half, u32 half_lcut, u32 p, u32 len) {
+    return (half && len <= half_lcut) ? half[p >> 1] : fsrc[p];
+}
 __host__ __device__ __forceinline__ u32 owner_rem_bits_for(u32 z, u32 cap) {
     u32 b = 0;
     while (b < cap && (((u64)z + 1) >> (31 - b)) == 0) ++b;
@@ -95,9 +99,11 @@
     if (threadIdx.x == 0) { u32 t = 0; for (int i = 0; i < OW_T / 64; ++i) t += sm[i]; tilecnt[blockIdx.x] = t; }
 }
 
+template <bool REC>
 __global__ __launch_bounds__(OW_T) void owner_build_kernel(const u32* __restrict__ flen, const u8* __restrict__ flen8, size_t n, const u32* __restrict__ tilebase,
                                                            u32* __restrict__ pos, u32* __restrict__ owner, uint2* __restrict__ cross,
-                                                           u8* __restrict__ cls, u32* __restrict__ lenl, const u32* __restrict__ rem_total, u32 rem_cap) {
+                                                           u8* __restrict__ cls, u32* __restrict__ lenl, const u32* __restrict__ rem_total, u32 rem_cap,
+                                                           uint4* __restrict__ rec, const u32* __restrict__ fsrc, const u32* __restrict__ half, u32 half_lcut) {
     __shared__ u32 s[OW_TILE + OW_TILE / 16 + 16];
     __shared__ u32 sm[OW_T / 64 + 1], smx[OW_T / 64];
     const size_t base = (size_t)blockIdx.x * OW_TILE;
@@ -159,7 +165,10 @@
         const u32 pl = l0 + k;
         if (f[k] != 0) {
             cur_start = pl + 1; cur_len = f[k]; cur_rank = rank++;
-            if (!stage_starts && base + pl < n) { pos[cur_rank] = (u32)(base + pl); if (lenl) lenl[cur_rank] = f[k]; }
+            if (!stage_starts && base + pl < n) {
+                pos[cur_rank] = (u32)(base + pl); if (lenl) lenl[cur_rank] = f[k];
+                if (REC) rec[cur_rank] = make_uint4((u32)(base + pl), f[k], factor_source(fsrc, half, half_lcut, (u32)(base + pl), f[k]), NOT_DONE);
+            }
         }
         const u32 d = pl - (cur_start - 1);
         out[k] = (cur_start != 0 && d < cur_len) ? (cur_rank | (min(cur_len - d - 1u, qmax) << rsh)) : NONE32;
@@ -200,7 +209,11 @@
         const u32 tb = tilebase[blockIdx.x];
         for (u32 e = threadIdx.x; e < total; e += OW_T) {
             const size_t p = base + s[e];
-            if (p < n) { pos[tb + e] = (u32)p; if (lenl) lenl[tb + e] = s[OW_TILE / 2 + e]; }
+            if (p < n) {
+                const u32 l = s[OW_TILE / 2 + e];
+                pos[tb + e] = (u32)p; if (lenl) lenl[tb + e] = l;
+                if (REC) rec[tb + e] = make_uint4((u32)p, l, factor_source(fsrc, half, half_lcut, (u32)p, l), NOT_DONE);
+            }
         }
     }
 }
@@ -218,34 +231,50 @@
     }
 }
 
+void half_sources_alive(const Ctx& c, const FactorSpace& fs) {
+    if (fs.half && (const char*)fs.half < c.arena.base + c.arena.top)
+        throw HipError{hipErrorUnknown, "the arena has grown into the half-indexed sources (FactorSpace::half) before the flatten records were written", (int)__LINE__};
+}
+
 void build_owner(Ctx& c, size_t n, FactorSpace& fs) {
     fs.have_list = false;
     fs.have_cls = false;
     fs.owner_rem_bits = 0;
+    fs.rec = nullptr;
     if (n == 0) return;
     const size_t mark = c.arena.mark();
     const u32 tiles = cdiv(n, OW_TILE);
+    const bool try_rec = fs.want_rec && fs.fpos && fs.flenl && fs.flen8 && !fs.src_prio;
+    const size_t rec_cap = try_rec ? n / 2 + 1 : 0;
+    uint4* rec = try_rec ? (uint4*)c.arena.alloc(rec_cap * sizeof(uint4)) : nullptr;
     u32* tilecnt = c.arena.get<u32>(tiles);
     uint2* cross = (uint2*)c.arena.alloc((size_t)tiles * sizeof(uint2));
     u32* pos = fs.fpos ? fs.fpos : c.arena.get<u32>(n);
     u32* d_total = c.arena.get<u32>(1);
+    if (try_rec) half_sources_alive(c, fs);
     {
         Ctx::ProfScope prof(c, K_EXTRACT, (u64)n * (fs.flen8 ? 1 : 4));
         owner_count_kernel<<<tiles, OW_T, 0, c.stream>>>(fs.flen, fs.flen8, n, tilecnt);
         LAUNCH_CHECK();
     }
     exclusive_sum_u32(c, tilecnt, tilecnt, tiles, d_total);
+    size_t z = try_rec ? (size_t)c.read(d_total) : 0;
+    const bool with_rec = try_rec && z <= rec_cap;
     {
-        Ctx::ProfScope prof(c, K_EXTRACT, (u64)n * (fs.flen8 ? 6 : 9));
+        Ctx::ProfScope prof(c, K_EXTRACT, (u64)n * (fs.flen8 ? 6 : 9) + (with_rec ? (u64)z * 20 : 0));
         const u32* rem_total = fs.want_owner_rem ? d_total : nullptr;
         const u32 rem_cap = std::min<u32>(fs.want_owner_rem, 8u);
-        owner_build_kernel<<<tiles, OW_T, 0, c.stream>>>(fs.flen, fs.flen8, n, tilecnt, pos, fs.owner, cross, fs.cls, fs.fpos ? fs.flenl : nullptr, rem_total, rem_cap);
+        if (with_rec) owner_build_kernel<true><<<tiles, OW_T, 0, c.stream>>>(fs.flen, fs.flen8, n, tilecnt, pos, fs.owner, cross, fs.cls, fs.flenl, rem_total, rem_cap,
+                                                                            rec, fs.fsrc, fs.half, fs.half_lcut);
+        else owner_build_kernel<false><<<tiles, OW_T, 0, c.stream>>>(fs.flen, fs.flen8, n, tilecnt, pos, fs.owner, cross, fs.cls, fs.fpos ? fs.flenl : nullptr, rem_total, rem_cap,
+                                                                     nullptr, nullptr, nullptr, 0u);
         LAUNCH_CHECK();
         owner_cross_kernel<<<tiles, 256, 0, c.stream>>>(cross, n, fs.owner, fs.cls, rem_total, rem_cap);
         fs.have_cls = fs.cls != nullptr;
         LAUNCH_CHECK();
     }
-    const size_t z = c.read(d_total);
+    if (!try_rec) z = c.read(d_total);
+    if (with_rec) { fs.rec = rec; fs.half = nullptr; }
     if (fs.fpos) { fs.nfact = z; fs.have_list = true; }
     fs.owner_rem_bits = fs.want_owner_rem ? owner_rem_bits_for((u32)z, std::min<u32>(fs.want_owner_rem, 8u)) : 0u;
     c.arena.release(mark);
@@ -290,8 +319,6 @@
     }
 }
 
-constexpr u32 NOT_DONE = 0xFFFFFFFFu;
-
 struct FlattenScalars { u32 waiting; u32 num_flattened; u32 max_depth; u32 pad; unsigned long long steps, waits; };
 
 __device__ __forceinline__ u32 lazy_source(const u32* __restrict__ prio, const u32* __restrict__ sa, size_t n, const u32* __restrict__ fsrc, u32 p) {
@@ -300,12 +327,13 @@
 }
 __global__ void flatten_init_kernel(const u32* __restrict__ fpos, size_t z, const u32* __restrict__ flen, const u32* __restrict__ orig,
                                     uint4* __restrict__ rec, const u32* __restrict__ lenl, const u32* __restrict__ src_prio,
-                                    const u32* __restrict__ src_sa, size_t src_n) {
+                                    const u32* __restrict__ src_sa, size_t src_n, const u32* __restrict__ half, u32 half_lcut) {
     const size_t i = (size_t)blockIdx.x * blockDim.x + threadIdx.x;
     if (i >= z) return;
     const u32 p = fpos[i];
-    const u32 o = src_prio ? lazy_source(src_prio, src_sa, src_n, orig, p) : orig[p];
-    rec[i] = make_uint4(p, lenl ? lenl[i] : flen[p], o, NOT_DONE);
+    const u32 l = lenl ? lenl[i] : flen[p];
+    const u32 o = src_prio ? lazy_source(src_prio, src_sa, src_n, orig, p) : factor_source(orig, half, half_lcut, p, l);
+    rec[i] = make_uint4(p, l, o, NOT_DONE);
 }
 __global__ void sources_fill_kernel(const u32* __restrict__ fpos, size_t z, const u32* __restrict__ src_prio, const u32* __restrict__ src_sa,
                                     size_t src_n, u32* fsrc) {
@@ -456,8 +484,12 @@
     FlattenScalars* d_sc = (FlattenScalars*)c.arena.alloc(sizeof(FlattenScalars));
     HIP_TRY(hipMemsetAsync(d_sc, 0, sizeof(FlattenScalars), s));
     const unsigned gz = cdiv(z, 256);
-    flatten_init_kernel<<<gz, 256, 0, s>>>(fpos, z, fs.flen, fs.fsrc, rec, fs.have_list ? fs.flenl : nullptr, fs.src_prio, fs.src_sa, fs.src_n);
-    LAUNCH_CHECK();
+    st->rec_from_build = rec_keep && fs.rec == rec_keep && fs.have_list;
+    if (!st->rec_from_build) {
+        half_sources_alive(c, fs);
+        flatten_init_kernel<<<gz, 256, 0, s>>>(fpos, z, fs.flen, fs.fsrc, rec, fs.have_list ? fs.flenl : nullptr, fs.src_prio, fs.src_sa, fs.src_n, fs.half, fs.half_lcut);
+        LAUNCH_CHECK();
+    }
     const size_t cmax = (z + K - 1) / K;
     uint4* work[2] = { (uint4*)c.arena.alloc(cmax * sizeof(uint4)), nullptr };
     u32 flat_growth = (u32)c.flatten_growth;
diff --git a/tudocomp_amd/csrc/stages.hpp b/tudocomp_amd/csrc/stages.hpp
--- a/tudocomp_amd/csrc/stages.hpp
+++ b/tudocomp_amd/csrc/stages.hpp
@@ -55,7 +55,13 @@
     const u32* src_prio = nullptr;
     const u32* src_sa = nullptr;
     size_t src_n = 0;
-};
+    bool want_half = false;
+    const u32* half = nullptr;
+    u32 half_lcut = 0;
+    bool want_rec = false;
+    void* rec = nullptr;
+};
+void half_sources_alive(const Ctx& c, const FactorSpace& fs);
 inline const u32* plain_owner(const FactorSpace& fs) {
     if (fs.owner_rem_bits) throw HipError{hipErrorUnknown, "owner[] carries remainder bits (FactorSpace::owner_rem_bits): this stage reads plain ranks", (int)__LINE__};
     return fs.owner;
@@ -82,7 +88,7 @@
 void factorize_max_heap(Ctx& c, size_t n, const u32* sa, const u32* isa, const u32* plcp, u32 maxlcp, u32 threshold, FactorSpace& fs,
                         FactorizeStats* st);
 
-struct FlattenStats { u64 num_flattened = 0; u64 max_depth_lb = 0; u32 rounds = 0; };
+struct FlattenStats { u64 num_flattened = 0; u64 max_depth_lb = 0; u32 rounds = 0; bool rec_from_build = false; };
 constexpr u32 FLATTEN_MAX_CHUNKS = 16;
 inline u32 flatten_chunk_count(u32 want, size_t z) { return (u32)std::max<size_t>(1, std::min<size_t>(std::min<size_t>(want, FLATTEN_MAX_CHUNKS), z)); }
 inline size_t flatten_chunk_start(size_t z, u32 k, u32 K) { return (size_t)((u64)z * k / K); }
@@ -96,7 +102,7 @@
 size_t encode_huff(Ctx& c, const u8* text, size_t n, FactorSpace fs, u8* d_out, size_t out_cap, EncodeStats* st);
 struct EncodeEarly;
 size_t encode_stream(Ctx& c, const u8* text, size_t n, FactorSpace fs, int coder, u8* d_out, size_t out_cap, EncodeStats* st, EncodeEarly* early = nullptr);
-EncodeEarly* encode_early_reserve(Ctx& c, size_t n, size_t z_rec = 0);
+EncodeEarly* encode_early_reserve(Ctx& c, size_t n, size_t z_rec = 0, const void* rec_placed = nullptr);
 void* encode_early_rec(EncodeEarly* e);
 void encode_early_run(Ctx& c, const u8* text, size_t n, FactorSpace fs, int coder, EncodeEarly* e, bool finish = true);
 void encode_early_free(EncodeEarly* e);
```

New measurement: 8964 MB/s, median of 6. No clear change (+0.7%).
